# Tencent/PocketFlow

Hardware: AMD Instinct MI355X
Metric: images/sec ResNet-50 INT8 quant-aware fine-tune (whole job; per GPU = value / n_gpus) (higher is better)
Workload: dtype bf16

## Files before the change

### include/pocketflow_hip.h

```cpp
#ifndef POCKETFLOW_HIP_H_
#define POCKETFLOW_HIP_H_

#include <stdint.h>

#ifdef __cplusplus
extern "C" {
#endif

enum { PF_F32 = 0, PF_BF16 = 1 };
enum { PF_ACT_NONE = 0, PF_ACT_RELU = 1, PF_ACT_RELU6 = 2 };
enum { PF_BUCKET_TENSOR = 0, PF_BUCKET_CHANNEL = 1, PF_BUCKET_SPLIT = 2 };

typedef struct PfSeg {
  int64_t offset;
  int64_t len;
  int32_t RS;
  int32_t layout;
  int32_t I, O;
  int32_t mode;
  int32_t bits;
  int32_t bucket_size;
  int32_t n_bucket;
  int64_t slot_offset;
  int64_t cb_offset;
// ... 17 lines not shown
                void* stream);

int pf_seg_minmax(const float* w_flat, const PfSeg* segs, const PfBlock* blocks, int n_blocks,
                  uint32_t* slots, void* stream);
int pf_seg_uq_apply(const float* w_flat, void* qw_flat, int out_dtype, const PfSeg* segs,
                    const PfBlock* blocks, int n_blocks, const uint32_t* slots, void* stream);

int pf_seg_nuq_apply(const float* w_flat, void* qw_flat, int out_dtype, uint8_t* idx_flat,
                     const float* codebooks, const PfSeg* segs, const PfBlock* blocks,
                     int n_blocks, const uint32_t* slots, void* stream);
int pf_seg_nuq_codebook_grad(const void* g_flat, int g_dtype, const uint8_t* idx_flat,
                             float* dcodebooks, int64_t* acc_ws, int64_t n_codebook, const PfSeg* segs,
                             const PfBlock* blocks, int n_blocks, const uint32_t* slots, void* stream);
int pf_seg_normalize(const float* w_flat, float* xn_out, const PfSeg* segs, int seg_index,
                     const uint32_t* slots, void* stream);

int pf_ws_bkup_merge_abs(const float* var, float* bkup, const float* mask, float* abs_out,
                         int64_t n, void* stream);
int pf_kth_largest_nonneg(const float* a, int64_t n, int64_t k_desc_index, float* out,
                          uint32_t* workspace, void* stream);
int pf_ws_mask_apply(float* var, const float* bkup, float* mask, const float* thr, int64_t n,
                     void* stream);
int pf_count_nonzero(const float* x, int64_t n, unsigned long long* out, void* stream);

int pf_cp_build_mask(float* mask, const uint8_t* keep_in, const uint8_t* keep_out, int O, int RS,
                     int I, void* stream);
int pf_cp_mask_grad(float* g, const uint8_t* keep_in, const uint8_t* keep_out, int O, int RS,
                    int I, void* stream);

int pf_adam_flat(float* p, const void* g, int g_dtype, float* m, float* v, const float* mask,
                 int64_t n, int64_t n_decay, float wd, float g_scale, float lr, float beta1,
                 float beta2, float eps, float beta1_power, float beta2_power, void* stream);
int pf_momentum_flat(float* p, const void* g, int g_dtype, float* acc, const float* mask,
                     int64_t n, int64_t n_decay, float wd, float g_scale, float lr, float momentum,
                     void* stream);
int pf_adam_flat_dev(float* p, const void* g, int g_dtype, float* m, float* v, const float* mask,
                     int64_t n, int64_t n_decay, float wd, float g_scale, const float* hp, float beta1,
                     float beta2, float eps, void* stream);
int pf_momentum_flat_dev(float* p, const void* g, int g_dtype, float* acc, const float* mask,
                         int64_t n, int64_t n_decay, float wd, float g_scale, const float* hp,
                         float momentum, void* stream);
int pf_set_floats(float* dst, float a, float b, float c, float d, void* stream);

int pf_ce_distill_fwd_bwd(const void* z_s, int zs_dtype, const float* labels, const void* z_t,
                          int zt_dtype, int B, int C, float tempr, float loss_w, float* losses,
                          void* dz_s, int dz_dtype, float* row_ws, void* stream);

int pf_bn_stats(const void* x, int dtype, int64_t rows, int C, float* partial ,
                int n_blocks, void* stream);
int pf_bn_finalize(const float* partial, int n_blocks, int64_t rows, int C, const void* x_row0,
                   int dtype, const float* gamma, const float* beta, float* moving_mean,
                   float* moving_var, float momentum, float eps, int training ,
                   int act, float* scale_shift , float* mean_invstd ,
                   uint32_t* slot , void* stream);
int pf_bn_act_quant_apply(const void* x, void* q, int dtype, int64_t rows, int C,
                          const float* scale_shift, int act, const uint32_t* slot, int bits,
                          int quantize, void* stream);
int pf_bn_bwd_stats(const void* dq, const void* x, int dtype, int64_t rows, int C,
                    const float* scale_shift, const float* mean_invstd, int act,
                    float* partial , int n_blocks, void* stream);
int pf_bn_bwd_finalize(const float* partial, int n_blocks, int C, float* dgamma, float* dbeta,
                       void* stream);
int pf_bn_bwd_apply(const void* dq, const void* x, void* dx, int dtype, int64_t rows, int C,
                    const float* scale_shift, const float* mean_invstd,
                    const float* dgamma, const float* dbeta, int act, void* stream);
int pf_bn_bwd_apply_add(const void* dq, const void* x, const void* addend, void* dx, int dtype,
                        int64_t rows, int C, const float* scale_shift, const float* mean_invstd,
                        const float* dgamma, const float* dbeta, int act, void* stream);
int pf_bn_eval_scale_shift(const float* gamma, const float* beta, const float* moving_mean,
                           const float* moving_var, float eps, int C, float* scale_shift,
                           void* stream);

int pf_conv1x1_stats_groups(int M, int N);
int pf_conv1x1_stats_groups_k(int M, int N, int K, int prologue);
int pf_conv1x1_fwd(const void* X, const void* W, void* Y, const void* R, const float* scale_shift,
                   int act, const uint32_t* slot, int bits, float* partial, int M, int N, int K,
                   int Ho, int Wo, int H, int Wd, int stride, int ymap, void* stream);
int pf_conv1x1_fwd_affine(const void* X, const void* W, void* Y, const float* scale_shift, int act,
                          const float* out_scale_shift, int out_act, int M, int N, int K, int Ho, int Wo, int H, int Wd,
                          int stride, void* stream);
int pf_conv1x1_bwd_data_bnstats(const void* dY, const void* Wt, void* dQ, const void* bn_x,
                                const float* bn_scale_shift, const float* bn_mean_invstd, int bn_act,
                                float* partial, int M, int N, int K, void* stream);
int pf_conv1x1_wrw_splits(int M, int N, int K);
int pf_conv1x1_wrw(const void* dY, const void* X, void* dW, int dw_dtype, float* workspace,
                   const float* scale_shift, int act, const uint32_t* slot, int bits, int M, int N,
                   int K, int Ho, int Wo, int H, int Wd, int stride, void* stream);

int pf_conv2d_stats_groups(int M, int N);
int pf_conv2d_stats_groups_geom(int imgs, int H, int Wd, int C, int N, int th, int tw, int stride, int pad_h, int pad_w,
                                int Ho, int Wo);
int pf_conv2d_fwd(const void* X, const void* W, void* Y, const void* zero, const void* R, float* partial,
                  const void* bn_x, const float* bn_scale_shift, const float* bn_mean_invstd, int bn_act,
                  int imgs, int H, int Wd, int C, int N, int th, int tw, int stride, int pad_h, int pad_w,
                  int Ho, int Wo, void* stream);
int pf_conv2d_fwd_affine(const void* X, const void* W, void* Y, const void* zero, const float* out_scale_shift, int out_act,
                         int imgs, int H, int Wd, int C, int N, int th, int tw, int stride, int pad_h, int pad_w, int Ho, int Wo,
                         void* stream);

int pf_conv2d_wrw_splits(int M, int N, int C, int taps);
int pf_conv2d_wrw(const void* dY, const void* X, void* dW, int dw_dtype, float* workspace, int imgs, int H, int Wd, int C,
                  int N, int th, int tw, int stride, int pad_h, int pad_w, int Ho, int Wo, void* stream);

typedef struct PfTransposeTile {
  int64_t src_off, dst_off;
  int32_t O, I, src_ld, dst_ld;
  int32_t o0, i0;
  int32_t reserved0, reserved1;
} PfTransposeTile;
int pf_seg_transpose(const void* src_flat, void* dst_flat, int dtype, const void* tiles, int n_tiles, void* stream);

int pf_maxpool_fwd(const void* x, void* y, void* idx, int dtype, int B, int H, int W, int C, int k, int stride,
                   int pad_h, int pad_w, int Ho, int Wo, void* stream);
int pf_maxpool_bwd(const void* dy, const void* idx, void* dx, int dtype, int B, int H, int W, int C, int k, int stride,
                   int pad_h, int pad_w, int Ho, int Wo, void* stream);

int pf_conv_stem_supported(int H, int Wd, int C, int N, int k, int stride, int pad);
int pf_conv_stem_fwd(const void* X, const void* W, void* Y, int imgs, int H, int Wd, void* stream);
int pf_conv_stem_wrw_slabs(int imgs, int H, int Wd);
int pf_conv_stem_wrw(const void* dY, const void* X, void* dW, int dw_dtype, float* workspace, int imgs, int H, int Wd,
                     void* stream);

int pf_conv_stem3_supported(int H, int Wd, int C, int N, int k, int stride, int pad_h, int pad_w, int Ho, int Wo);
int pf_conv_stem3_fwd(const void* X, const void* W, void* Y, int imgs, int H, int Wd, int N, int pad_h, int pad_w, int Ho, int Wo,
                      void* stream);
int pf_conv_stem3_wrw_slabs(int imgs, int H, int Wd, int N, int pad_h, int pad_w, int Ho, int Wo);
int pf_conv_stem3_wrw(const void* dY, const void* X, void* dW, int dw_dtype, float* workspace, int imgs, int H, int Wd, int N,
                      int pad_h, int pad_w, int Ho, int Wo, void* stream);

int pf_depthwise_supported(int C, int k, int stride);
int pf_depthwise_groups(int B, int Ho, int Wo, int C);
int pf_depthwise_fwd(const void* X, const void* W, void* Y, int dtype, float* partial, int B, int H, int Wd, int C, int k,
                     int stride, int pad_h, int pad_w, int Ho, int Wo, void* stream);
int pf_depthwise_bwd_data(const void* dY, const void* W, void* dX, int dtype, int B, int H, int Wd, int C, int k,
                          int stride, int pad_h, int pad_w, int Ho, int Wo, void* stream);
int pf_depthwise_wrw(const void* dY, const void* X, void* dW, int dtype, int dw_dtype, float* slabs, int B, int H, int Wd,
                     int C, int k, int stride, int pad_h, int pad_w, int Ho, int Wo, void* stream);

typedef struct PfImageDesc {
  int64_t offset;
  int32_t h, w;
  float scale_y, scale_x;
  int32_t off_y, off_x;
  int32_t flip;
  int32_t reserved;
} PfImageDesc;
int pf_image_resize_bilinear(const void* src, const PfImageDesc* desc, void* out, int out_dtype, int B, int OH,
                             int OW, float mean_r, float mean_g, float mean_b, void* stream);

int pf_conv2d_bwd_data_strided(const void* dY, const void* Wt, void* dX, const void* zero, int imgs, int H, int Wd, int C, int N,
                               int R, int S, int stride, int pad_h, int pad_w, int Ho, int Wo, void* stream);
int pf_conv2d_bwd_data_strided_stats_groups(int imgs, int H, int Wd, int C, int stride);
int pf_conv2d_bwd_data_strided_bnstats(const void* dY, const void* Wt, void* dX, const void* zero, const void* bn_x,
                                       const float* bn_scale_shift, const float* bn_mean_invstd, int bn_act, float* partial,
                                       int imgs, int H, int Wd, int C, int N, int R, int S, int stride, int pad_h, int pad_w,
                                       int Ho, int Wo, void* stream);

int pf_convg_small_splits(int M, int Nc, int K);
int pf_convg_fwd(const void* x, const void* w, const float* bias, void* y, int dtype, int imgs, int H, int W, int C, int N, int R,
                 int S, int stride, int pad_h, int pad_w, int Ho, int Wo, float* slab, int64_t slab_elems, void* stream);
int pf_convg_bwd_data(const void* dy, const void* w, void* dx, int dtype, int imgs, int H, int W, int C, int N, int R, int S,
                      int stride, int pad_h, int pad_w, int Ho, int Wo, float* slab, int64_t slab_elems, void* stream);
int pf_convg_wrw_splits(int imgs, int C, int N, int R, int S, int Ho, int Wo);
int pf_convg_wrw(const void* dy, const void* x, void* dw, int dtype, int dw_dtype, float* slab, int imgs, int H, int W, int C, int N,
                 int R, int S, int stride, int pad_h, int pad_w, int Ho, int Wo, void* stream);

// ... 32 lines not shown
```

### pocketflow_amd/csrc/pf_conv.hip

```cpp
#include "pf_conv_common.h"

template <int BN_T, bool PRO, bool BWD, bool MAP>
__global__ __launch_bounds__(PF_THREADS, 2) void k_conv1x1_fwd(const ConvArgs a) {
  constexpr int WM = (BN_T == 128) ? 64 : 32;
  constexpr int JM = WM / 16;
  constexpr int CS_LD = BN_T + 8;
  constexpr int VPR = BN_T / 8;
  constexpr int RPP = PF_THREADS / VPR;
  constexpr int NBV = BN_T * 8 / PF_THREADS;
  constexpr int A_EL = CV_BM * CV_LDK, B_EL = BN_T * CV_LDK;
  constexpr int C_EL = CV_BM * CS_LD;
  constexpr int RED_FL = 4 * RPP * BN_T;
  constexpr int SM_BYTES_AB = (A_EL + B_EL) * 2;
  constexpr int SM_BYTES = SM_BYTES_AB > RED_FL * 4 ? (SM_BYTES_AB > C_EL * 2 ? SM_BYTES_AB : C_EL * 2)
                                                    : RED_FL * 4;
  constexpr int SS_BYTES = PRO ? 2 * CV_MAXK * 4 : 0;
  __shared__ __attribute__((aligned(16))) unsigned char smem[SM_BYTES + SS_BYTES];
  float* ssl = reinterpret_cast<float*>(smem + SM_BYTES);
  __shared__ float bpl[BWD ? 4 * BN_T : 4];
  bf16_t* As = reinterpret_cast<bf16_t*>(smem);
  bf16_t* Bs = As + A_EL;
  bf16_t* Cs = reinterpret_cast<bf16_t*>(smem);
  float* red = reinterpret_cast<float*>(smem);

// ... 165 lines not shown
      const int rl = wrow + p * RPP;
      const int m = m0 + rl, n = n0 + wvec * 8;
      if (m < a.M && n < a.N) {
        uint4 c = *reinterpret_cast<const uint4*>(Cs + rl * CS_LD + wvec * 8);
        const int64_t orow = (MAP && a.ymap) ? map_row(a, m) : (int64_t)m;
        if (bwd_stats) {
          float f[8], xv[8];
          unpack8(c, f);
          unpack8(rres[p], xv);
          const float* bp = bpl + wvec * 8;
#pragma unroll
          for (int j = 0; j < 8; ++j) {
            const float u = fmaf(bp[j], xv[j], bp[BN_T + j]);
            const float dy = (u > a.b_lo && u < a.b_hi) ? f[j] : 0.f;
            st_s[j] += dy;
            st_q[j] = fmaf(dy, (xv[j] - bp[2 * BN_T + j]) * bp[3 * BN_T + j], st_q[j]);
          }
        } else if (a.R != nullptr || a.partial != nullptr) {
          float f[8];
          unpack8(c, f);
          if (a.partial != nullptr) {
#pragma unroll
            for (int j = 0; j < 8; ++j) {
              st_s[j] += f[j];
              st_q[j] = fmaf(f[j], f[j], st_q[j]);
              st_mn[j] = pf_acc_min(st_mn[j], f[j]);
              st_mx[j] = pf_acc_max(st_mx[j], f[j]);
            }
          }
        }
        *reinterpret_cast<uint4*>(a.Y + orow * a.N + n) = c;
      }
    }
    __syncthreads();
  };

  for (int it = 0; it < total; it += 2) {
    body(it, ra0, av0);
    if (it + 1 < total) body(it + 1, ra1, av1);
  }

  if (a.partial != nullptr) {
    __syncthreads();
#pragma unroll
    for (int j = 0; j < 8; ++j) {
      red[(0 * RPP + wrow) * BN_T + wvec * 8 + j] = st_s[j];
      red[(1 * RPP + wrow) * BN_T + wvec * 8 + j] = st_q[j];
      red[(2 * RPP + wrow) * BN_T + wvec * 8 + j] = st_mn[j];
      red[(3 * RPP + wrow) * BN_T + wvec * 8 + j] = st_mx[j];
    }
    __syncthreads();
    const int nstat = bwd_stats ? 2 : 4;
    for (int t = tid; t < nstat * BN_T; t += PF_THREADS) {
      const int stat = t / BN_T, c = t - stat * BN_T;
      float v = red[(stat * RPP) * BN_T + c];
      for (int r = 1; r < RPP; ++r) {
        const float w = red[(stat * RPP + r) * BN_T + c];
        v = (stat < 2) ? (v + w) : (stat == 2 ? fminf(v, w) : fmaxf(v, w));
      }
      if (n0 + c < a.N) a.partial[((int64_t)g * nstat + stat) * a.N + n0 + c] = v;
    }
  }
}

#include <stdlib.h>
static int conv_bn_of(int N) {
  if (pf_tuning().conv_bn == 64) return 64;
  return (N % 128 == 0) ? 128 : 64;
}

static int conv_fwd_grid(int tiles_m, int tiles_n, int* G_out) {
  int G = 512 / tiles_n;
  G = (G / 8) * 8;
  if (G < 8) G = 8;
  const int need = ((tiles_m + 7) / 8) * 8;
  if (G > need) G = need;
  *G_out = G;
  return G * tiles_n;
}

int pf_conv_stream_plan(int M, int N, int K, int* nw_out);
int pf_conv_stream_groups(int nsplit);
int pf_conv_stream_launch(const ConvArgs& a, bool pro, bool bwd, hipStream_t st);

extern "C" int pf_conv1x1_stats_groups(int M, int N) {
  const int bn = conv_bn_of(N);
  int G;
  conv_fwd_grid((M + CV_BM - 1) / CV_BM, (N + bn - 1) / bn, &G);
  return G;
}

extern "C" int pf_conv2d_stats_groups(int M, int N);
int pf_igemm_stats_groups(int M, int N, int pro);
int pf_igemm_conv1x1(const void* X, const void* W, void* Y, const void* R, float* partial, const void* bn_x,
                     const float* bss, const float* bmi, float b_lo, float b_hi, const float* scale_shift,
                     const uint32_t* slot, float kq, float act_lo, float act_hi, int M, int N, int K, int Ho, int Wo,
                     int H, int Wd, int stride, const float* oss, int oact, hipStream_t st, int ymap = 0);
#ifndef PF_CONV_IGEMM_PLAIN_MINK
#define PF_CONV_IGEMM_PLAIN_MINK 256
#endif
static bool conv_use_igemm(bool pro, int K) {
  if ((pro ? pf_tuning().conv_igemm_pro : pf_tuning().conv_igemm) == 0) return false;
  return (K % 64) == 0 && (pro || K >= PF_CONV_IGEMM_PLAIN_MINK);
}

extern "C" int pf_conv1x1_stats_groups_k(int M, int N, int K, int prologue) {
  int nw = 0;
  const int nsplit = pf_conv_stream_plan(M, N, K, &nw);
  if (nsplit > 0) return pf_conv_stream_groups(nsplit);
  if (conv_use_igemm(prologue != 0, K)) return pf_igemm_stats_groups(M, N, prologue != 0);
  return pf_conv1x1_stats_groups(M, N);
}

static int conv_fwd_launch(const void* X, const void* W, void* Y, const void* R, const float* scale_shift,
                           int act, const uint32_t* slot, int bits, float* partial, int M, int N, int K,
                           int Ho, int Wo, int H, int Wd, int stride, int ymap, const void* bx,
                           const float* bss, const float* bmi, int bact, void* stream, const float* oss = nullptr,
                           int oact = PF_ACT_NONE) {
  if (oss != nullptr && (R != nullptr || partial != nullptr || bx != nullptr || ymap)) return (int)hipErrorInvalidValue;
  if (M <= 0 || N <= 0 || K <= 0 || (K % 8) || (N % 8)) return (int)hipErrorInvalidValue;
  if (!pf_aligned16(X) || !pf_aligned16(W) || !pf_aligned16(Y) || (R && !pf_aligned16(R)))
    return (int)hipErrorInvalidValue;
  if (slot != nullptr && (bits < 1 || bits > 32 || scale_shift == nullptr)) return (int)hipErrorInvalidValue;
  if (scale_shift != nullptr && K > CV_MAXK) return (int)hipErrorInvalidValue;
  if (stride < 1 || (stride > 1 && (Ho <= 0 || Wo <= 0 || H <= 0 || Wd <= 0))) return (int)hipErrorInvalidValue;
  ConvArgs a;
  a.X = (const bf16_t*)X; a.W = (const bf16_t*)W; a.Y = (bf16_t*)Y; a.R = (const bf16_t*)R;
  a.ss = scale_shift; a.slot = slot; a.partial = partial;
  a.kq = uq_k_of_bits(slot ? bits : 8);
  a.act_lo = (act == PF_ACT_NONE) ? -INFINITY : 0.0f;
  a.act_hi = (act == PF_ACT_RELU6) ? 6.0f : INFINITY;
  a.M = M; a.N = N; a.K = K;
  a.Ho = Ho; a.Wo = Wo; a.H = H; a.Wd = Wd; a.stride = stride; a.ymap = ymap; a.rows_per_split = 0;
  a.bx = (const bf16_t*)bx; a.bss = bss; a.bmi = bmi;
  a.b_lo = (bact == PF_ACT_NONE) ? -INFINITY : 0.0f;
  a.b_hi = (bact == PF_ACT_RELU6) ? 6.0f : INFINITY;
  a.oss = oss; a.oact = oact;
  if (bx != nullptr && (R != nullptr || partial == nullptr || bss == nullptr || bmi == nullptr || stride != 1 ||
                        !pf_aligned16(bx)))
    return (int)hipErrorInvalidValue;
  const int bn = conv_bn_of(N);
  a.tiles_m = (M + CV_BM - 1) / CV_BM;
  a.tiles_n = (N + bn - 1) / bn;
  const int grid = conv_fwd_grid(a.tiles_m, a.tiles_n, &a.G);
  hipStream_t st = (hipStream_t)stream;
  const bool pro = scale_shift != nullptr;
  if (bx != nullptr && pro) return (int)hipErrorInvalidValue;
  {
    const int r = pf_conv_stream_launch(a, pro, bx != nullptr, st);
    if (r >= 0) return r;
  }
  if (!ymap && conv_use_igemm(pro, K)) {
    const int r = pf_igemm_conv1x1(X, W, Y, R, partial, bx, bss, bmi, a.b_lo, a.b_hi, scale_shift, slot, a.kq, a.act_lo,
                                   a.act_hi, M, N, K, Ho, Wo, H, Wd, stride, oss, oact, st);
    if (r >= 0) return r;
  }
  if (ymap && stride > 1 && !pro && bx == nullptr && R == nullptr && partial == nullptr && oss == nullptr && conv_use_igemm(false, K) &&
      (N % 64) == 0) {
    const int r = pf_igemm_conv1x1(X, W, Y, nullptr, nullptr, nullptr, nullptr, nullptr, a.b_lo, a.b_hi, nullptr, nullptr, a.kq, a.act_lo,
                                   a.act_hi, M, N, K, Ho, Wo, H, Wd, stride, nullptr, PF_ACT_NONE, st, 1);
    if (r >= 0) return r;
  }
  if (oss != nullptr) {
    const int r = conv_fwd_launch(X, W, Y, R, scale_shift, act, slot, bits, partial, M, N, K, Ho, Wo, H, Wd, stride, ymap, bx, bss,
                                  bmi, bact, stream);
    if (r != 0) return r;
    return pf_bn_act_quant_apply(Y, Y, PF_BF16, M, N, oss, oact, nullptr, 8, 0, stream);
  }
  const bool map = stride != 1;
#define PF_CV(BNV)                                                                             \
  do {                                                                                         \
    if (pro) { if (map) k_conv1x1_fwd<BNV, true, false, true><<<grid, PF_THREADS, 0, st>>>(a);  \
               else k_conv1x1_fwd<BNV, true, false, false><<<grid, PF_THREADS, 0, st>>>(a); }   \
    else if (bx != nullptr) k_conv1x1_fwd<BNV, false, true, false><<<grid, PF_THREADS, 0, st>>>(a); \
    else { if (map) k_conv1x1_fwd<BNV, false, false, true><<<grid, PF_THREADS, 0, st>>>(a);     \
           else k_conv1x1_fwd<BNV, false, false, false><<<grid, PF_THREADS, 0, st>>>(a); }      \
  } while (0)
  if (bn == 128) PF_CV(128); else PF_CV(64);
#undef PF_CV
  PF_LAUNCH_CHECK();
  return 0;
}

extern "C" int pf_conv1x1_fwd(const void* X, const void* W, void* Y, const void* R, const float* scale_shift,
                              int act, const uint32_t* slot, int bits, float* partial, int M, int N, int K,
                              int Ho, int Wo, int H, int Wd, int stride, int ymap, void* stream) {
  return conv_fwd_launch(X, W, Y, R, scale_shift, act, slot, bits, partial, M, N, K, Ho, Wo, H, Wd, stride, ymap,
                         nullptr, nullptr, nullptr, PF_ACT_NONE, stream);
}

extern "C" int pf_conv1x1_fwd_affine(const void* X, const void* W, void* Y, const float* scale_shift, int act,
                                     const float* out_scale_shift, int out_act, int M, int N, int K, int Ho, int Wo, int H,
                                     int Wd, int stride, void* stream) {
  if (out_scale_shift == nullptr) return (int)hipErrorInvalidValue;
  return conv_fwd_launch(X, W, Y, nullptr, scale_shift, act, nullptr, 8, nullptr, M, N, K, Ho, Wo, H, Wd, stride, 0,
                         nullptr, nullptr, nullptr, PF_ACT_NONE, stream, out_scale_shift, out_act);
}

extern "C" int pf_conv1x1_bwd_data_bnstats(const void* dY, const void* Wt, void* dQ, const void* bn_x,
                                           const float* bn_scale_shift, const float* bn_mean_invstd, int bn_act,
                                           float* partial, int M, int N, int K, void* stream) {
  return conv_fwd_launch(dY, Wt, dQ, nullptr, nullptr, PF_ACT_NONE, nullptr, 8, partial, M, K, N, 0, 0, 0, 0, 1, 0,
                         bn_x, bn_scale_shift, bn_mean_invstd, bn_act, stream);
}

#define WR_TN 128
#define WR_TK 64
#define WR_BM 64
#define WR_LDM (WR_BM + 8)

__device__ __forceinline__ void st_transposed(bf16_t* S, int c0, int m, const uint4& v) {
  const uint32_t w[4] = {v.x, v.y, v.z, v.w};
  const int mg = m >> 3, ml = m & 7;
#pragma unroll
  for (int j = 0; j < 8; ++j) {
    const int c = c0 + j;
    S[c * WR_LDM + (((mg ^ ((c >> 3) & 7)) << 3) | ml)] = (bf16_t)((w[j >> 1] >> ((j & 1) * 16)) & 0xFFFFu);
  }
}

template <bool PRO>
__global__ __launch_bounds__(PF_THREADS, 2) void k_conv1x1_wrw(const ConvArgs a) {
  __shared__ __attribute__((aligned(16))) bf16_t Ds[WR_TN * WR_LDM];
  __shared__ __attribute__((aligned(16))) bf16_t Qs[WR_TK * WR_LDM];
  const int ntile = gridDim.x, nwg = gridDim.x * gridDim.y;
  int wg = blockIdx.y * gridDim.x + blockIdx.x;
  {
    const int xcd = wg & 7, idx = wg >> 3;
    const int q = nwg >> 3, r = nwg & 7;
    wg = (xcd < r ? xcd * (q + 1) : r * (q + 1) + (xcd - r) * q) + idx;
  }
  const int tile = wg % ntile, split = wg / ntile;
  const int tn = tile % a.tiles_n, tk = tile / a.tiles_n;
  const int n0 = tn * WR_TN, k0 = tk * WR_TK;
  const int mbeg = split * a.rows_per_split;
  const int mend = (mbeg + a.rows_per_split < a.M) ? (mbeg + a.rows_per_split) : a.M;
  const int tid = threadIdx.x, wave = tid >> 6, lane = tid & 63;
  const int frow = lane & 15, fm = lane >> 4;

  Pro pro;
  pro_init(pro, a.act_lo, a.act_hi, a.kq, PRO ? a.slot : nullptr);
  const int qkp = tid & 7;
  if (PRO) {
    const int k = k0 + qkp * 8;
    if (k < a.K) {
#pragma unroll
      for (int j = 0; j < 8; ++j) { pro.sc[j] = pro_fold_scale(pro, a.ss[k + j]); pro.sh[j] = pro_fold_shift(pro, a.ss[a.K + k + j]); }
    }
  }
  f32x4 acc[2][4];
#pragma unroll
  for (int i = 0; i < 2; ++i)
#pragma unroll
    for (int j = 0; j < 4; ++j) acc[i][j] = (f32x4){0.f, 0.f, 0.f, 0.f};

  uint4 rd[4], rq[2];
  bool vq[2];
  auto gload = [&](int mb) {
#pragma unroll
    for (int i = 0; i < 4; ++i) {
      const int p = tid + i * PF_THREADS;
      const int m = mb + (p >> 4), n = n0 + (p & 15) * 8;
      uint4 v = make_uint4(0, 0, 0, 0);
      if (m < mend && n < a.N) v = *reinterpret_cast<const uint4*>(a.W + (int64_t)m * a.N + n);
      rd[i] = v;
    }
#pragma unroll
    for (int i = 0; i < 2; ++i) {
      const int p = tid + i * PF_THREADS;
      const int m = mb + (p >> 3), k = k0 + (p & 7) * 8;
      uint4 v = make_uint4(0, 0, 0, 0);
      vq[i] = (m < mend && k < a.K);
      if (vq[i]) v = *reinterpret_cast<const uint4*>(a.X + map_row(a, m) * a.K + k);
      rq[i] = v;
    }
  };
  auto sstore = [&]() {
#pragma unroll
    for (int i = 0; i < 4; ++i) {
      const int p = tid + i * PF_THREADS;
      st_transposed(Ds, (p & 15) * 8, p >> 4, rd[i]);
    }
#pragma unroll
    for (int i = 0; i < 2; ++i) {
      const int p = tid + i * PF_THREADS;
      uint4 v = rq[i];
// ... 151 lines not shown
```

### pocketflow_amd/csrc/pf_conv_common.h

```cpp
#pragma once
#include "pf_common.h"

typedef __attribute__((ext_vector_type(8))) __bf16 bf16x8;
typedef __attribute__((ext_vector_type(4))) float f32x4;

#define CV_BM 128
#define CV_BK 64
#define CV_LDK (CV_BK + 8)
#define CV_MAXK 2048

typedef __attribute__((ext_vector_type(2))) __bf16 bf16x2_t;
typedef __attribute__((ext_vector_type(2))) float f32x2_t;
__device__ __forceinline__ uint32_t pack_bf16x2(float a, float b) {
  const f32x2_t v = {a, b};
  const bf16x2_t r = __builtin_convertvector(v, bf16x2_t);
  return *reinterpret_cast<const uint32_t*>(&r);
}
__device__ __forceinline__ void unpack8(const uint4& v, float* o) {
  o[0] = __uint_as_float(v.x << 16); o[1] = __uint_as_float(v.x & 0xFFFF0000u);
  o[2] = __uint_as_float(v.y << 16); o[3] = __uint_as_float(v.y & 0xFFFF0000u);
  o[4] = __uint_as_float(v.z << 16); o[5] = __uint_as_float(v.z & 0xFFFF0000u);
  o[6] = __uint_as_float(v.w << 16); o[7] = __uint_as_float(v.w & 0xFFFF0000u);
}
__device__ __forceinline__ uint4 pack8(const float* o) {
  return make_uint4(pack_bf16x2(o[0], o[1]), pack_bf16x2(o[2], o[3]), pack_bf16x2(o[4], o[5]),
                    pack_bf16x2(o[6], o[7]));
}

struct ConvArgs {
  const bf16_t* X;
  const bf16_t* W;
  bf16_t* Y;
  const bf16_t* R;
  const float* ss;
  const uint32_t* slot;
  float* partial;
  float kq, act_lo, act_hi;
  int M, N, K;
  int tiles_m, tiles_n, G;
  int Ho, Wo, H, Wd, stride;
  int ymap;
  int rows_per_split;
  const bf16_t* bx;
  const float* bss;
  const float* bmi;
  float b_lo, b_hi;
  const float* oss;
  int oact;
};

__device__ __forceinline__ uint4 out_affine8(const uint4& c, const float* __restrict__ oss, int N, int n, int act) {
  float f[8];
  unpack8(c, f);
  const float4 s0 = *reinterpret_cast<const float4*>(oss + n), s1 = *reinterpret_cast<const float4*>(oss + n + 4);
  const float4 h0 = *reinterpret_cast<const float4*>(oss + N + n), h1 = *reinterpret_cast<const float4*>(oss + N + n + 4);
  const float sc[8] = {s0.x, s0.y, s0.z, s0.w, s1.x, s1.y, s1.z, s1.w};
  const float sh[8] = {h0.x, h0.y, h0.z, h0.w, h1.x, h1.y, h1.z, h1.w};
#pragma unroll
  for (int j = 0; j < 8; ++j) {
    float y = fmaf(sc[j], f[j], sh[j]);
    if (act != PF_ACT_NONE) y = fmaxf(y, 0.f);
    if (act == PF_ACT_RELU6) y = fminf(y, 6.f);
    f[j] = y;
  }
  return pack8(f);
}

__device__ __forceinline__ int64_t map_row(const ConvArgs& a, int m) {
  if (a.stride == 1) return m;
  const int hw = a.Ho * a.Wo;
  const int n = m / hw, rem = m - n * hw;
  const int ho = rem / a.Wo, wo = rem - ho * a.Wo;
  return ((int64_t)n * a.H + (int64_t)ho * a.stride) * a.Wd + (int64_t)wo * a.stride;
}

struct Pro {
  float sc[8], sh[8];
  float lo, hi;
  float beta, c1, c2;
  int quant;
};
__device__ __forceinline__ void pro_init(Pro& p, float act_lo, float act_hi, float kq, const uint32_t* slot) {
  p.quant = 0; p.beta = 0.f; p.c1 = 1.f; p.c2 = 1.f;
  if (slot != nullptr) {
    float alpha, beta;
    slot_alpha_beta(slot, alpha, beta);
    p.quant = 1; p.beta = beta; p.c1 = kq / alpha; p.c2 = alpha / kq;
  }
  p.lo = (act_lo - p.beta) * p.c1;
  p.hi = (act_hi - p.beta) * p.c1;
}
__device__ __forceinline__ float pro_fold_scale(const Pro& p, float scale) { return scale * p.c1; }
__device__ __forceinline__ float pro_fold_shift(const Pro& p, float shift) { return (shift - p.beta) * p.c1; }
__device__ __forceinline__ float pro_point(const Pro& p, float sc, float sh, float x) {
  const float t = __builtin_amdgcn_fmed3f(fmaf(sc, x, sh), p.lo, p.hi);
  return p.quant ? fmaf(rintf(t), p.c2, p.beta) : t;
}
__device__ __forceinline__ uint4 pro_apply_scalar(const Pro& p, const uint4& v) {
  float f[8];
  unpack8(v, f);
#pragma unroll
  for (int j = 0; j < 8; ++j) f[j] = pro_point(p, p.sc[j], p.sh[j], f[j]);
  return pack8(f);
}
typedef float f32x2p_t __attribute__((ext_vector_type(2)));
__device__ __forceinline__ uint4 pro_apply(const Pro& p, const uint4& v) {
  const uint32_t w[4] = {v.x, v.y, v.z, v.w};
  uint32_t o[4];
  if (p.quant) {
    const f32x2p_t c2 = {p.c2, p.c2}, be = {p.beta, p.beta};
#pragma unroll
    for (int i = 0; i < 4; ++i) {
      const f32x2p_t x = {__uint_as_float(w[i] << 16), __uint_as_float(w[i] & 0xFFFF0000u)};
      const f32x2p_t sc = {p.sc[2 * i], p.sc[2 * i + 1]}, sh = {p.sh[2 * i], p.sh[2 * i + 1]};
      const f32x2p_t t = __builtin_elementwise_fma(sc, x, sh);
      const f32x2p_t r = {rintf(__builtin_amdgcn_fmed3f(t[0], p.lo, p.hi)), rintf(__builtin_amdgcn_fmed3f(t[1], p.lo, p.hi))};
      const f32x2p_t q = __builtin_elementwise_fma(r, c2, be);
      o[i] = pack_bf16x2(q[0], q[1]);
    }
  } else {
#pragma unroll
    for (int i = 0; i < 4; ++i) {
      const f32x2p_t x = {__uint_as_float(w[i] << 16), __uint_as_float(w[i] & 0xFFFF0000u)};
      const f32x2p_t sc = {p.sc[2 * i], p.sc[2 * i + 1]}, sh = {p.sh[2 * i], p.sh[2 * i + 1]};
      const f32x2p_t t = __builtin_elementwise_fma(sc, x, sh);
      o[i] = pack_bf16x2(__builtin_amdgcn_fmed3f(t[0], p.lo, p.hi), __builtin_amdgcn_fmed3f(t[1], p.lo, p.hi));
    }
  }
  return make_uint4(o[0], o[1], o[2], o[3]);
}

__device__ __forceinline__ uint32_t lds_addr(const void* p) { return (uint32_t)(uintptr_t)p; }
// ... 57 lines not shown
```

### pocketflow_amd/csrc/pf_conv_stream.hip

```cpp
#include "pf_conv_common.h"
#include <stdlib.h>

#define ST_THREADS 512
#define ST_WAVES 8
#define ST_GRID 256

template <int NW, bool PRO, bool BWD, bool MAP, bool AFF = false>
__global__ __launch_bounds__(ST_THREADS) void k_conv1x1_stream(const ConvArgs a, const int nsplit) {
  constexpr int JM = (NW == 256) ? 1 : 2;
  constexpr int RS = 16 * JM;
  constexpr int NI = NW / 16;
  constexpr int D = (NW == 128) ? 2 : 4;
  constexpr int CS_LD = NW + 8;
  constexpr int VPR = NW / 8;
  constexpr int RPP = 64 / VPR;
  constexpr int NP = RS / RPP;
  constexpr int NR = 2 * JM;

  extern __shared__ __attribute__((aligned(16))) unsigned char smem[];
  const int K = a.K, KC = K >> 6, KV = K >> 3;
  bf16_t* Wl = reinterpret_cast<bf16_t*>(smem);
  float* aux = reinterpret_cast<float*>(smem + (size_t)NW * K * 2);
  const int aux_fl = PRO ? 2 * K : (BWD ? 4 * NW : 0);
  bf16_t* Cs_all = reinterpret_cast<bf16_t*>(smem + (size_t)NW * K * 2 + (size_t)aux_fl * 4);
  float* red = reinterpret_cast<float*>(Cs_all);

  const int tid = threadIdx.x, wave = tid >> 6, lane = tid & 63;
  const int l15 = lane & 15, q = lane >> 4;
  bf16_t* Cs = Cs_all + wave * (RS * CS_LD);

  const int xcd = blockIdx.x & 7, idx = blockIdx.x >> 3;
  const int slice = idx % nsplit, g = (idx / nsplit) * 8 + xcd;
  const int nsets = gridDim.x / nsplit;
  const int n0 = slice * NW;
  const int sstep = nsets * ST_WAVES;
  const int NS = (a.M + RS - 1) / RS;
  const int s_first = g * ST_WAVES + wave;
  const int cnt = (s_first < NS) ? (NS - s_first + sstep - 1) / sstep : 0;
  const int T = cnt * KC;

  Pro pro;
  pro_init(pro, a.act_lo, a.act_hi, a.kq, PRO ? a.slot : nullptr);
  {
    const int swz_mask = (KV >= 16) ? 15 : 7;
    for (int v = tid; v < NW * KV; v += ST_THREADS) {
      const int n = v / KV, c = v - n * KV;
      uint4 w = make_uint4(0, 0, 0, 0);
      if (n0 + n < a.N) w = *reinterpret_cast<const uint4*>(a.W + (int64_t)(n0 + n) * K + c * 8);
      *reinterpret_cast<uint4*>(Wl + ((int64_t)n * KV + (c ^ (n & swz_mask))) * 8) = w;
    }
    if (PRO) for (int i = tid; i < 2 * K; i += ST_THREADS)
      aux[i] = (i < K) ? pro_fold_scale(pro, a.ss[i]) : pro_fold_shift(pro, a.ss[i]);
    if (BWD) for (int i = tid; i < 4 * NW; i += ST_THREADS) {
      const int qq = i / NW, c = n0 + (i - qq * NW);
      float v = 0.f;
      if (c < a.N) v = (qq < 2) ? a.bss[qq * a.N + c] : a.bmi[(qq - 2) * a.N + c];
      aux[i] = v;
    }
  }
  __syncthreads();

  const int wswz = (KV >= 16) ? l15 : (l15 & 7);
  const bf16_t* __restrict__ side = BWD ? a.bx : nullptr;
  const bool has_r = !BWD && a.R != nullptr;
  const int wvec = lane % VPR, wrow = lane / VPR;

  f32x4 acc[NI][JM];
  uint4 ring[D][NR];
  uint4 rres[NP];
  uint2 rr[NI][JM];
  float st_s[8], st_q[8], st_mn[8], st_mx[8];
#pragma unroll
  for (int j = 0; j < 8; ++j) { st_s[j] = 0.f; st_q[j] = 0.f; st_mn[j] = INFINITY; st_mx[j] = -INFINITY; }

  int ld_s = s_first, ld_kc = 0;
  auto issue = [&](uint4 (&r)[NR]) {
#pragma unroll
    for (int j = 0; j < JM; ++j) {
      int m = ld_s * RS + j * 16 + l15;
      m = (m < a.M) ? m : (a.M - 1);
      const int64_t row = (!MAP || a.ymap) ? (int64_t)m : map_row(a, m);
      const bf16_t* p = a.X + row * K + ld_kc * 64 + q * 8;
      r[j * 2 + 0] = *reinterpret_cast<const uint4*>(p);
      r[j * 2 + 1] = *reinterpret_cast<const uint4*>(p + 32);
    }
    if (++ld_kc == KC) { ld_kc = 0; ld_s += sstep; }
  };
  auto issue_side = [&](int s, int p) {
    const int m = s * RS + p * RPP + wrow, n = n0 + wvec * 8;
    uint4 v = make_uint4(0, 0, 0, 0);
    if (m < a.M && n < a.N) {
      const int64_t orow = (MAP && a.ymap) ? map_row(a, m) : (int64_t)m;
      v = *reinterpret_cast<const uint4*>(side + orow * a.N + n);
    }
    rres[p] = v;
  };

  auto issue_res = [&](int s) {
#pragma unroll
    for (int j = 0; j < JM; ++j) {
      const int m = s * RS + j * 16 + l15;
      const int64_t orow = (m < a.M) ? ((MAP && a.ymap) ? map_row(a, m) : (int64_t)m) : 0;
#pragma unroll
      for (int i = 0; i < NI; ++i) {
        const int n = n0 + i * 16 + q * 4;
        uint2 v = make_uint2(0, 0);
        if (m < a.M && n < a.N) v = *reinterpret_cast<const uint2*>(a.R + orow * a.N + n);
        rr[i][j] = v;
      }
    }
  };
#pragma clang loop unroll(full)
  for (int d = 0; d < D; ++d)
    if (d < T) issue(ring[d]);
  if (has_r && cnt > 0) issue_res(s_first);
  if (side != nullptr && cnt > 0) {
#pragma unroll
    for (int p = 0; p < NP; ++p) issue_side(s_first, p);
  }

  int cs = s_first, ckc = 0;
  int slot = 0;
  for (int t = 0; t < T; ++t) {
    uint4 v[NR];
    const bool refill = t + D < T;
#pragma clang loop unroll(full)
    for (int d = 0; d < D; ++d) {
      if (slot == d) {
#pragma unroll
        for (int i = 0; i < NR; ++i) v[i] = ring[d][i];
        if (refill) issue(ring[d]);
      }
    }
    slot = (slot + 1 == D) ? 0 : slot + 1;
    if (ckc == 0) {
#pragma unroll
      for (int i = 0; i < NI; ++i)
#pragma unroll
        for (int j = 0; j < JM; ++j) acc[i][j] = (f32x4){0.f, 0.f, 0.f, 0.f};
    }
#pragma unroll
    for (int kk = 0; kk < 2; ++kk) {
      if (PRO) {
        const int k = ckc * 64 + kk * 32 + q * 8;
        const float4 s0 = *reinterpret_cast<const float4*>(aux + k), s1 = *reinterpret_cast<const float4*>(aux + k + 4);
        const float4 h0 = *reinterpret_cast<const float4*>(aux + K + k), h1 = *reinterpret_cast<const float4*>(aux + K + k + 4);
        pro.sc[0] = s0.x; pro.sc[1] = s0.y; pro.sc[2] = s0.z; pro.sc[3] = s0.w;
        pro.sc[4] = s1.x; pro.sc[5] = s1.y; pro.sc[6] = s1.z; pro.sc[7] = s1.w;
        pro.sh[0] = h0.x; pro.sh[1] = h0.y; pro.sh[2] = h0.z; pro.sh[3] = h0.w;
        pro.sh[4] = h1.x; pro.sh[5] = h1.y; pro.sh[6] = h1.z; pro.sh[7] = h1.w;
      }
      bf16x8 xf[JM];
#pragma unroll
      for (int j = 0; j < JM; ++j) {
        uint4 u = v[j * 2 + kk];
        if (PRO) u = (NW == 128) ? pro_apply_scalar(pro, u) : pro_apply(pro, u);
        xf[j] = *reinterpret_cast<const bf16x8*>(&u);
      }
      const int c = (ckc * 8 + kk * 4 + q) ^ wswz;
      constexpr int WB = 4;
#pragma unroll
      for (int ib = 0; ib < NI; ib += WB) {
        bf16x8 wf[WB];
#pragma unroll
        for (int i = 0; i < WB; ++i)
          wf[i] = *reinterpret_cast<const bf16x8*>(Wl + ((int64_t)((ib + i) * 16 + l15) * KV + c) * 8);
#pragma unroll
        for (int i = 0; i < WB; ++i)
#pragma unroll
          for (int j = 0; j < JM; ++j)
            acc[ib + i][j] = __builtin_amdgcn_mfma_f32_16x16x32_bf16(wf[i], xf[j], acc[ib + i][j], 0, 0, 0);
      }
      if (PRO) __builtin_amdgcn_sched_group_barrier(0x100, 4, 0);
      constexpr int DEPTH = (NW == 128) ? 2 : 4;
      __builtin_amdgcn_sched_group_barrier(0x100, DEPTH, 0);
#pragma unroll
      for (int i = 0; i < NI - DEPTH; ++i) {
        __builtin_amdgcn_sched_group_barrier(0x008, JM, 0);
        __builtin_amdgcn_sched_group_barrier(0x100, 1, 0);
      }
      __builtin_amdgcn_sched_group_barrier(0x008, DEPTH * JM, 0);
    }
    const bool last = (ckc == KC - 1);
    const int s = cs;
    if (++ckc == KC) { ckc = 0; cs += sstep; }
    if (!last) continue;

    if (has_r) {
#pragma unroll
      for (int i = 0; i < NI; ++i)
#pragma unroll
        for (int j = 0; j < JM; ++j) {
          acc[i][j][0] += __uint_as_float(rr[i][j].x << 16); acc[i][j][1] += __uint_as_float(rr[i][j].x & 0xFFFF0000u);
          acc[i][j][2] += __uint_as_float(rr[i][j].y << 16); acc[i][j][3] += __uint_as_float(rr[i][j].y & 0xFFFF0000u);
        }
    }
#pragma unroll
    for (int i = 0; i < NI; ++i)
#pragma unroll
      for (int j = 0; j < JM; ++j) {
        const uint2 w = make_uint2(pack_bf16x2(acc[i][j][0], acc[i][j][1]), pack_bf16x2(acc[i][j][2], acc[i][j][3]));
        *reinterpret_cast<uint2*>(Cs + (j * 16 + l15) * CS_LD + i * 16 + q * 4) = w;
      }
    const bool more = (cs < NS);
    if (has_r && more) issue_res(cs);
    float bpr[32];
    if (BWD && NW != 128) {
#pragma unroll
      for (int qq = 0; qq < 4; ++qq)
#pragma unroll
        for (int j = 0; j < 8; ++j) bpr[qq * 8 + j] = aux[qq * NW + wvec * 8 + j];
    } else if (BWD) {
#pragma unroll
      for (int i = 0; i < 32; ++i) bpr[i] = 0.f;
    }
    constexpr int CB = (NW == 128) ? 1 : 4;
    uint4 cv[CB];
#pragma unroll
    for (int p = 0; p < NP; ++p) {
      const int rl = p * RPP + wrow;
      const int m = s * RS + rl, n = n0 + wvec * 8;
      if (p % CB == 0) {
#pragma unroll
        for (int pb = 0; pb < CB; ++pb)
          if (p + pb < NP) cv[pb] = *reinterpret_cast<const uint4*>(Cs + ((p + pb) * RPP + wrow) * CS_LD + wvec * 8);
      }
      uint4 c = cv[p % CB];
      const uint4 sv = rres[p];
      if (side != nullptr && more) issue_side(cs, p);
      if (m < a.M && n < a.N) {
        const int64_t orow = (MAP && a.ymap) ? map_row(a, m) : (int64_t)m;
        if (BWD) {
          float f[8], xv[8];
          unpack8(c, f);
          unpack8(sv, xv);
          const float* bp = (NW == 128) ? (aux + wvec * 8) : bpr;
          constexpr int BPS = (NW == 128) ? NW : 8;
#pragma unroll
          for (int j = 0; j < 8; ++j) {
            const float u = fmaf(bp[j], xv[j], bp[BPS + j]);
            const float dy = (u > a.b_lo && u < a.b_hi) ? f[j] : 0.f;
            st_s[j] += dy;
            st_q[j] = fmaf(dy, (xv[j] - bp[2 * BPS + j]) * bp[3 * BPS + j], st_q[j]);
          }
        } else if (a.R != nullptr || a.partial != nullptr) {
          float f[8];
          unpack8(c, f);
          if (a.partial != nullptr) {
#pragma unroll
            for (int j = 0; j < 8; ++j) {
              st_s[j] += f[j];
              st_q[j] = fmaf(f[j], f[j], st_q[j]);
              st_mn[j] = pf_acc_min(st_mn[j], f[j]);
              st_mx[j] = pf_acc_max(st_mx[j], f[j]);
            }
          }
        }
        if constexpr (AFF) c = out_affine8(c, a.oss, a.N, n, a.oact);
        *reinterpret_cast<uint4*>(a.Y + orow * a.N + n) = c;
      }
    }
  }

  if (a.partial != nullptr) {
#pragma unroll
    for (int o = VPR; o < 64; o <<= 1) {
#pragma unroll
      for (int j = 0; j < 8; ++j) {
        st_s[j] += __shfl_xor(st_s[j], o, 64);
        st_q[j] += __shfl_xor(st_q[j], o, 64);
        st_mn[j] = fminf(st_mn[j], __shfl_xor(st_mn[j], o, 64));
        st_mx[j] = fmaxf(st_mx[j], __shfl_xor(st_mx[j], o, 64));
      }
    }
    __syncthreads();
    if (lane < VPR) {
#pragma unroll
      for (int j = 0; j < 8; ++j) {
        red[(0 * ST_WAVES + wave) * NW + lane * 8 + j] = st_s[j];
        red[(1 * ST_WAVES + wave) * NW + lane * 8 + j] = st_q[j];
        red[(2 * ST_WAVES + wave) * NW + lane * 8 + j] = st_mn[j];
        red[(3 * ST_WAVES + wave) * NW + lane * 8 + j] = st_mx[j];
      }
    }
    __syncthreads();
    const int nstat = BWD ? 2 : 4;
    for (int t = tid; t < nstat * NW; t += ST_THREADS) {
      const int stat = t / NW, c = t - stat * NW;
      float v = red[(stat * ST_WAVES) * NW + c];
      for (int w = 1; w < ST_WAVES; ++w) {
        const float x = red[(stat * ST_WAVES + w) * NW + c];
        v = (stat < 2) ? (v + x) : (stat == 2 ? fminf(v, x) : fmaxf(v, x));
      }
      if (n0 + c < a.N) a.partial[((int64_t)g * nstat + stat) * a.N + n0 + c] = v;
    }
  }
}

static int stream_enabled() {
  return pf_tuning().conv_stream;
}

static int stream_max_split() {
  return pf_tuning().conv_stream_maxsplit;
}

int pf_conv_stream_plan(int M, int N, int K, int* nw_out) {
  if (!stream_enabled()) return 0;
  if ((K % 64) || K > 512 || (N % 64) || N > 2048) return 0;
  if (M < 4096) return 0;
  int nsplit = 1;
  while ((int64_t)(N / nsplit) * K > 32768 || N / nsplit > 256) nsplit *= 2;
  const int nw = N / nsplit;
  if (nsplit > stream_max_split() || (ST_GRID % (8 * nsplit)) || (nw != 64 && nw != 128 && nw != 256)) return 0;
  if (nsplit >= 2 && N < 4 * K) return 0;
  *nw_out = nw;
  return nsplit;
}

int pf_conv_stream_groups(int nsplit) { return ST_GRID / nsplit; }

template <int NW, bool PRO, bool BWD, bool MAP, bool AFF = false>
static int stream_launch_t(const ConvArgs& a, int nsplit, hipStream_t st) {
  const int JM = (NW == 256) ? 1 : 2, RS = 16 * JM;
  const size_t aux_fl = PRO ? 2 * (size_t)a.K : (BWD ? 4 * (size_t)NW : 0);
  const size_t lds = (size_t)NW * a.K * 2 + aux_fl * 4 + (size_t)ST_WAVES * RS * (NW + 8) * 2;
  if (int e = pf_require_lds(reinterpret_cast<const void*>(&k_conv1x1_stream<NW, PRO, BWD, MAP, AFF>), lds)) return e;
  k_conv1x1_stream<NW, PRO, BWD, MAP, AFF><<<ST_GRID, ST_THREADS, lds, st>>>(a, nsplit);
  PF_LAUNCH_CHECK();
  return 0;
}

int pf_conv_stream_launch(const ConvArgs& a, bool pro, bool bwd, hipStream_t st) {
  int nw = 0;
  const int nsplit = pf_conv_stream_plan(a.M, a.N, a.K, &nw);
  if (nsplit == 0) return -1;
  const bool map = a.stride != 1;
  if (a.oss != nullptr) {
    if (map || bwd) return -1;
#define PF_STA(NWV) do { return pro ? stream_launch_t<NWV, true, false, false, true>(a, nsplit, st)     \
                                    : stream_launch_t<NWV, false, false, false, true>(a, nsplit, st); } while (0)
    if (nw == 64) PF_STA(64);
    if (nw == 128) PF_STA(128);
    PF_STA(256);
#undef PF_STA
  }
#define PF_ST(NWV)                                                                                  \
  do {                                                                                              \
    if (pro) return map ? stream_launch_t<NWV, true, false, true>(a, nsplit, st)                    \
                        : stream_launch_t<NWV, true, false, false>(a, nsplit, st);                  \
    if (bwd) return stream_launch_t<NWV, false, true, false>(a, nsplit, st);                        \
    return map ? stream_launch_t<NWV, false, false, true>(a, nsplit, st)                            \
               : stream_launch_t<NWV, false, false, false>(a, nsplit, st);                          \
  } while (0)
  if (nw == 64) PF_ST(64);
  if (nw == 128) PF_ST(128);
  PF_ST(256);
#undef PF_ST
}
```

### pocketflow_amd/csrc/pf_igemm.h

```cpp
#pragma once
#include "pf_conv_common.h"

#define LDS_PTR(p) ((__attribute__((address_space(3))) void*)(p))

#if defined(__HIP_DEVICE_COMPILE__)
typedef __amdgpu_buffer_rsrc_t pf_rsrc_t;
#define PF_MAKE_RSRC(p, bytes) __builtin_amdgcn_make_buffer_rsrc((void*)(p), (short)0, (int)(bytes), 0x00020000)
#define PF_BUFFER_LOAD_LDS16(rs, lds, voff, soff) __builtin_amdgcn_raw_ptr_buffer_load_lds(rs, LDS_PTR(lds), 16, voff, soff, 0, 0)
#else
typedef int pf_rsrc_t;
#define PF_MAKE_RSRC(p, bytes) 0
#define PF_BUFFER_LOAD_LDS16(rs, lds, voff, soff) ((void)(rs), (void)(lds), (void)(voff), (void)(soff))
#endif

struct IgArgs {
  const bf16_t* X;
  const bf16_t* W;
  bf16_t* Y;
  const bf16_t* zero;
  uint32_t x_bytes, w_bytes;
  const bf16_t* R;
  float* partial;
  const bf16_t* bx;
  const float* bss;
  const float* bmi;
  float b_lo, b_hi;
  const float* ss;
  const uint32_t* slot;
  float kq, act_lo, act_hi;
  int M, N, C;
  int th, tw;
  int H, Wd, Ho, Wo, stride, pad_h, pad_w;
  int tiles_m, tiles_n, G;
  int w_r0, w_rs, w_s0, w_ss, w_S, w_taps_full;
  int o_sub, o_y, o_x, o_H, o_W;
  const float* oss;
  int oact;
};

template <int N> __device__ __forceinline__ void wait_vm() { asm volatile("s_waitcnt vmcnt(%0)" ::"n"(N) : "memory"); }

#define IG_PLAIN 0
#define IG_BWD 1
#define IG_PRO 2
```

### pocketflow_amd/csrc/pf_igemm.hip

```cpp
#include "pf_conv_common.h"
#include <stdio.h>
#include <stdlib.h>

#include "pf_igemm.h"

#ifndef PF_IG_ABLATE
#define PF_IG_ABLATE 0
#endif
#define PF_IG_NO_DMA (PF_IG_ABLATE == 2 || PF_IG_ABLATE == 3 || PF_IG_ABLATE == 4)
#define PF_IG_FAKE_FRAGS (PF_IG_ABLATE == 3 || PF_IG_ABLATE == 4)

#ifdef PF_IG_TIMING
#define PF_IG_STAMP(k) do { if (tm_tile == 2) tmk[k] = (uint32_t)__builtin_readcyclecounter(); } while (0)
#else
#define PF_IG_STAMP(k) do { } while (0)
#endif

#ifdef PF_IG_CODES
#define PF_IG_XB 1
__device__ __forceinline__ bf16x8 ig_codes_to_bf16x8(uint2 c) {
  uint32_t r[4];
#pragma unroll
  for (int h = 0; h < 2; ++h) {
    const uint32_t w = h ? c.y : c.x;
    const float f0 = (float)(w & 0xffu), f1 = (float)((w >> 8) & 0xffu), f2 = (float)((w >> 16) & 0xffu), f3 = (float)(w >> 24);
    r[h * 2 + 0] = __builtin_amdgcn_perm(__float_as_uint(f1), __float_as_uint(f0), 0x07060302u);
    r[h * 2 + 1] = __builtin_amdgcn_perm(__float_as_uint(f3), __float_as_uint(f2), 0x07060302u);
  }
  const uint4 u = make_uint4(r[0], r[1], r[2], r[3]);
  return *reinterpret_cast<const bf16x8*>(&u);
}
#else
#define PF_IG_XB 2
#endif

template <int BM, int BN, int WM, int WN, int NS, int MODE, bool SUB = false, bool AFF = false>
__global__ __launch_bounds__(64 * WM * WN) void k_igemm(const IgArgs a) {
  constexpr bool BWD = (MODE == IG_BWD), PRO = (MODE == IG_PRO);
  static_assert(!PRO || NS == 2 || NS == 3, "the in-LDS prologue pass is written for the 2- and 3-stage rings");
  constexpr bool PRO3 = PRO && NS == 3;
  constexpr int NWC = WM * WN;
  constexpr int T = 64 * NWC;
  constexpr int TS = T;
  constexpr int TE = T;
  constexpr int WR = BM / WM, WC = BN / WN;
  constexpr int JM = WR / 16, NI = WC / 16;
  constexpr int XB = PF_IG_XB;
  constexpr int ACH = 4 * XB, AROW = 64 * XB;
  constexpr int AS = BM * ACH / TS, BS = BN * 8 / TS;
  constexpr int A_BYTES = BM * AROW, B_BYTES = BN * 128, STAGE = A_BYTES + B_BYTES;
  constexpr int CS_LD = BN + 8, CS_LD_B = BN + 8;
  constexpr int VPR = BN / 8, RPP = TE / VPR, NP = BM / RPP;
  static_assert(AS >= 1 && BS >= 1 && NP >= 1, "tile too small for the block");
  constexpr int LPS = AS + BS;
  extern __shared__ __attribute__((aligned(16))) unsigned char smem[];
  bf16_t* Cs = reinterpret_cast<bf16_t*>(smem);
  float* red = reinterpret_cast<float*>(smem);
  constexpr int RING_B = NS * STAGE, CT_B = BM * CS_LD_B * 2;
  float* bpl = reinterpret_cast<float*>(smem + (RING_B > CT_B ? RING_B : CT_B));
  float* ssl = bpl;

  const int tid = threadIdx.x, lane = tid & 63;
  const int wave = __builtin_amdgcn_readfirstlane(tid >> 6);
  const int swave = wave;
  const int cwave = wave % NWC;
  const int wm = cwave / WN, wn = cwave % WN;
  const int l15 = lane & 15, q = lane >> 4;
  const int srow = (swave * 64 + lane) >> 3;
  const int schunk = (lane & 7) ^ ((lane >> 3) & 7);
  const int srowA = (XB == 2) ? srow : ((swave * 64 + lane) >> 2);
  const int schunkA = (XB == 2) ? schunk : ((lane & 3) ^ ((lane >> 4) & 3));

  const int xcd = blockIdx.x & 7, L = blockIdx.x >> 3;
  const int g = xcd + 8 * (L / a.tiles_n), tn = L % a.tiles_n;
  const int n0 = tn * BN;
  const int cch = a.C >> 6;
  const int taps = a.th * a.tw;
  const int nk = taps * cch;
  const int64_t wrow = (int64_t)(SUB ? a.w_taps_full : taps) * a.C;
  const int hw_o = a.Ho * a.Wo;

  if (BWD) {
    for (int i = tid; i < 4 * BN; i += T) {
      const int qq = i / BN, c = n0 + (i - qq * BN);
      float v = 0.f;
      if (c < a.N) v = (qq < 2) ? a.bss[qq * a.N + c] : a.bmi[(qq - 2) * a.N + c];
      bpl[i] = v;
    }
  }

  float st_s[8], st_q[8], st_mn[8], st_mx[8];
#pragma unroll
  for (int j = 0; j < 8; ++j) { st_s[j] = 0.f; st_q[j] = 0.f; st_mn[j] = INFINITY; st_mx[j] = -INFINITY; }
  const int wvec = tid % VPR, wrw = tid / VPR;
  const bf16_t* __restrict__ side = BWD ? a.bx : nullptr;
  Pro pro;
  pro_init(pro, a.act_lo, a.act_hi, a.kq, PRO ? a.slot : nullptr);
  if (PRO3) {
    for (int i = tid; i < 2 * a.C; i += T) ssl[i] = (i < a.C) ? pro_fold_scale(pro, a.ss[i]) : pro_fold_shift(pro, a.ss[i]);
    __syncthreads();
  }

  const pf_rsrc_t rsX = PF_MAKE_RSRC(a.X, a.x_bytes);
  const pf_rsrc_t rsW = PF_MAKE_RSRC(a.W, a.w_bytes);
  constexpr uint32_t OOB = 0x80000000u;
  uint32_t boff[BS];
#pragma unroll
  for (int i = 0; i < BS; ++i) {
    const int n = n0 + i * (TS / 8) + srow;
    boff[i] = (n < a.N) ? (uint32_t)(((int64_t)n * wrow + schunk * 8) * 2) : OOB;
  }

  const bool pointwise = a.th == 1 && a.tw == 1 && a.stride == 1 && a.pad_h == 0 && a.pad_w == 0 && a.Ho == a.H && a.Wo == a.Wd;
  constexpr bool XPRE = !BWD && NS == 3 && 2 * STAGE >= BM * CS_LD_B * 2;
  constexpr int RB0 = XPRE ? 2 : 0;
  uint32_t pbase[AS], pmask[AS];
  int s_r = 0, s_s = 0, s_cc = 0, s_ks = 0, s_tap = 0;
  auto setup_tile = [&](int m0) {
#pragma unroll
    for (int i = 0; i < AS; ++i) {
      const int m = m0 + i * (TS / ACH) + srowA;
      pbase[i] = 0; pmask[i] = 0;
      if (pointwise) {
        if (m < a.M) { pbase[i] = (uint32_t)(m * a.C + schunkA * (16 / XB)) * (uint32_t)XB; pmask[i] = 1u; }
      } else if (m < a.M) {
        const int img = m / hw_o, rem = m - img * hw_o;
        const int ho = rem / a.Wo, wo = rem - ho * a.Wo;
        const int h0 = ho * a.stride - a.pad_h, w0 = wo * a.stride - a.pad_w;
        pbase[i] = (uint32_t)(((img * a.H + h0) * a.Wd + w0) * a.C + schunkA * (16 / XB)) * (uint32_t)XB;
        uint32_t mk = 0;
        for (int r = 0; r < a.th; ++r)
          for (int sx = 0; sx < a.tw; ++sx)
            if ((unsigned)(h0 + r) < (unsigned)a.H && (unsigned)(w0 + sx) < (unsigned)a.Wd) mk |= 1u << (r * a.tw + sx);
        pmask[i] = mk;
      }
    }
    s_r = 0; s_s = 0; s_cc = 0; s_ks = 0; s_tap = 0;
  };
  auto stage = [&](int buf) {
    unsigned char* As = smem + buf * STAGE;
    unsigned char* Bs = As + A_BYTES;
    const uint32_t tapoff = (uint32_t)(((s_r * a.Wd + s_s) * a.C + s_cc * 64) * XB);
#if !PF_IG_NO_DMA
#pragma unroll
    for (int i = 0; i < AS; ++i) {
      const uint32_t voff = ((pmask[i] >> s_tap) & 1u) ? (pbase[i] + tapoff) : OOB;
      PF_BUFFER_LOAD_LDS16(rsX, As + (i * (TS / ACH) + swave * (64 / ACH)) * AROW, voff, 0);
    }
    uint32_t woff = (uint32_t)(s_ks * 128);
    if constexpr (SUB) woff = (uint32_t)((((a.w_r0 + s_r * a.w_rs) * a.w_S + a.w_s0 + s_s * a.w_ss) * a.C + s_cc * 64) * 2);
#pragma unroll
    for (int i = 0; i < BS; ++i)
      PF_BUFFER_LOAD_LDS16(rsW, Bs + (i * (TS / 8) + swave * 8) * 128, boff[i], woff);
#else
    (void)As; (void)Bs; (void)tapoff;
#endif
    ++s_ks;
    if (++s_cc == cch) { s_cc = 0; ++s_tap; if (++s_s == a.tw) { s_s = 0; ++s_r; } }
  };
  bool pre = false;
#ifdef PF_IG_TIMING
  uint32_t tmk[16];
  int tm_tile = -1;
#pragma unroll
  for (int k = 0; k < 16; ++k) tmk[k] = 0;
#endif
  for (int tm = g; tm < a.tiles_m; tm += a.G) {
    const int m0 = tm * BM;
#ifdef PF_IG_TIMING
    ++tm_tile;
#endif
    PF_IG_STAMP(0);
    if (!pre) setup_tile(m0);

    f32x4 acc[NI][JM];
#pragma unroll
    for (int i = 0; i < NI; ++i)
#pragma unroll
      for (int j = 0; j < JM; ++j) acc[i][j] = (f32x4){0.f, 0.f, 0.f, 0.f};
    uint2 rr[NI][JM];
    const bool has_r = !BWD && a.R != nullptr;
    constexpr bool RPRE = BM * BN <= 128 * 256;
    auto load_residual = [&]() {
#pragma unroll
      for (int j = 0; j < JM; ++j) {
        const int m = m0 + wm * WR + j * 16 + l15;
#pragma unroll
        for (int i = 0; i < NI; ++i) {
          const int n = n0 + wn * WC + i * 16 + q * 4;
          rr[i][j] = make_uint2(0, 0);
          if (m < a.M && n < a.N) rr[i][j] = *reinterpret_cast<const uint2*>(a.R + (int64_t)m * a.N + n);
        }
      }
    };
    auto add_residual = [&](auto& c) {
#pragma unroll
      for (int j = 0; j < JM; ++j)
#pragma unroll
        for (int i = 0; i < NI; ++i) {
          c[i][j][0] += __uint_as_float(rr[i][j].x << 16); c[i][j][1] += __uint_as_float(rr[i][j].x & 0xFFFF0000u);
          c[i][j][2] += __uint_as_float(rr[i][j].y << 16); c[i][j][3] += __uint_as_float(rr[i][j].y & 0xFFFF0000u);
        }
    };

    int ibuf = RB0;
    float4 ps0 = make_float4(0, 0, 0, 0), ps1 = ps0, ph0 = ps0, ph1 = ps0;
    auto fetch_ss = [&](int cc) {
      const float* p = a.ss + cc * 64 + schunk * 8;
      ps0 = *reinterpret_cast<const float4*>(p); ps1 = *reinterpret_cast<const float4*>(p + 4);
      ph0 = *reinterpret_cast<const float4*>(p + a.C); ph1 = *reinterpret_cast<const float4*>(p + a.C + 4);
    };
    auto transform3 = [&](int buf, int cc, int i0, int i1) {
      const uint32_t pss = lds_addr(ssl + cc * 64 + schunk * 8);
      float4 s0, s1, h0, h1;
      if (i1 - i0 == 1 || i1 - i0 == 2) {
        const uint32_t pd = lds_addr(smem + buf * STAGE + srow * 128 + (lane & 7) * 16) + (uint32_t)(i0 * (TS / 8) * 128);
        uint4 v0, v1 = make_uint4(0, 0, 0, 0);
        if (i1 - i0 == 1) lds_read_b128x4_1(pss, pss + (uint32_t)a.C * 4u, pd, s0, s1, h0, h1, v0);
        else lds_read_b128x4_2(pss, pss + (uint32_t)a.C * 4u, pd, pd + (TS / 8) * 128, s0, s1, h0, h1, v0, v1);
        pro.sc[0] = s0.x; pro.sc[1] = s0.y; pro.sc[2] = s0.z; pro.sc[3] = s0.w;
        pro.sc[4] = s1.x; pro.sc[5] = s1.y; pro.sc[6] = s1.z; pro.sc[7] = s1.w;
        pro.sh[0] = h0.x; pro.sh[1] = h0.y; pro.sh[2] = h0.z; pro.sh[3] = h0.w;
        pro.sh[4] = h1.x; pro.sh[5] = h1.y; pro.sh[6] = h1.z; pro.sh[7] = h1.w;
        lds_write_b128(pd, pro_apply(pro, v0));
        if (i1 - i0 == 2) lds_write_b128(pd + (TS / 8) * 128, pro_apply(pro, v1));
        return;
      }
      lds_read_b128x4(pss, pss + (uint32_t)a.C * 4u, s0, s1, h0, h1);
      pro.sc[0] = s0.x; pro.sc[1] = s0.y; pro.sc[2] = s0.z; pro.sc[3] = s0.w;
      pro.sc[4] = s1.x; pro.sc[5] = s1.y; pro.sc[6] = s1.z; pro.sc[7] = s1.w;
      pro.sh[0] = h0.x; pro.sh[1] = h0.y; pro.sh[2] = h0.z; pro.sh[3] = h0.w;
      pro.sh[4] = h1.x; pro.sh[5] = h1.y; pro.sh[6] = h1.z; pro.sh[7] = h1.w;
      const uint32_t pv = lds_addr(smem + buf * STAGE + srow * 128 + (lane & 7) * 16);
      static_assert(!PRO3 || AS == 1 || AS == 2 || AS == 4 || AS == 8, "vector count per lane");
#pragma unroll
      for (int i = 0; i < AS; i += 2) {
        if (i >= i0 && i < i1) {
          if (i + 1 < i1) {
            uint4 v0, v1;
            lds_read_b128x2(pv + i * (TS / 8) * 128, pv + (i + 1) * (TS / 8) * 128, v0, v1);
            lds_write_b128(pv + i * (TS / 8) * 128, pro_apply(pro, v0));
            lds_write_b128(pv + (i + 1) * (TS / 8) * 128, pro_apply(pro, v1));
          } else {
            lds_write_b128(pv + i * (TS / 8) * 128, pro_apply(pro, lds_read_b128(pv + i * (TS / 8) * 128)));
          }
        } else if (i + 1 >= i0 && i + 1 < i1) {
          lds_write_b128(pv + (i + 1) * (TS / 8) * 128, pro_apply(pro, lds_read_b128(pv + (i + 1) * (TS / 8) * 128)));
        }
      }
    };
    auto transform = [&](int buf) {
      const float rs[8] = {ps0.x, ps0.y, ps0.z, ps0.w, ps1.x, ps1.y, ps1.z, ps1.w};
      const float rh[8] = {ph0.x, ph0.y, ph0.z, ph0.w, ph1.x, ph1.y, ph1.z, ph1.w};
#pragma unroll
      for (int j = 0; j < 8; ++j) { pro.sc[j] = pro_fold_scale(pro, rs[j]); pro.sh[j] = pro_fold_shift(pro, rh[j]); }
      unsigned char* As = smem + buf * STAGE;
#pragma unroll
      for (int i = 0; i < AS; ++i) {
        uint4* p = reinterpret_cast<uint4*>(As + (i * (TS / 8) + srow) * 128 + (lane & 7) * 16);
        *p = pro_apply(pro, *p);
      }
    };
    {
#pragma unroll
    for (int d = 0; d < NS - 1; ++d)
      if (d < nk) {
        if (d > 0 || !pre) {
          if (PRO && !PRO3) fetch_ss(s_cc);
          stage(ibuf);
        }
        ibuf = (ibuf + 1 == NS) ? 0 : ibuf + 1;
      }
    PF_IG_STAMP(1);
    if (nk >= NS - 1) wait_vm<(NS - 2) * LPS>(); else wait_vm<0>();
// ... 22 lines not shown
#pragma unroll
      for (int kk = 0; kk < 2; ++kk) {
        const int coff = (((kk * 4 + q) ^ (l15 & 7)) << 4);
        bf16x8 wf[NI], xf[JM];
#if PF_IG_ABLATE != 1
#if PF_IG_FAKE_FRAGS
#pragma unroll
        for (int i = 0; i < NI; ++i) { uint4 u = make_uint4(lane, i, kk, 0x3f803f80u); asm volatile("" : "+v"(u.x)); wf[i] = *reinterpret_cast<const bf16x8*>(&u); }
#pragma unroll
        for (int j = 0; j < JM; ++j) { uint4 u = make_uint4(lane, j, kk, 0x3f803f80u); asm volatile("" : "+v"(u.x)); xf[j] = *reinterpret_cast<const bf16x8*>(&u); }
        (void)coff;
#else
#pragma unroll
        for (int i = 0; i < NI; ++i)
          wf[i] = *reinterpret_cast<const bf16x8*>(Bs + (wn * WC + i * 16 + l15) * 128 + coff);
#ifdef PF_IG_CODES
        const int coffA = ((((kk * 2 + (q >> 1)) ^ ((l15 >> 2) & 3)) << 4) + (q & 1) * 8);
#pragma unroll
        for (int j = 0; j < JM; ++j)
          xf[j] = ig_codes_to_bf16x8(*reinterpret_cast<const uint2*>(As + (wm * WR + j * 16 + l15) * AROW + coffA));
#else
#pragma unroll
        for (int j = 0; j < JM; ++j)
          xf[j] = *reinterpret_cast<const bf16x8*>(As + (wm * WR + j * 16 + l15) * 128 + coff);
#endif
#endif
#pragma unroll
        for (int i = 0; i < NI; ++i)
#pragma unroll
          for (int j = 0; j < JM; ++j)
            acc[i][j] = __builtin_amdgcn_mfma_f32_16x16x32_bf16(wf[i], xf[j], acc[i][j], 0, 0, 0);
        if constexpr (NI == 4 && JM == 4 && PRO3) {
          __builtin_amdgcn_sched_group_barrier(0x100, NI + JM, 0);
          __builtin_amdgcn_sched_group_barrier(0x008, NI * JM, 0);
        }
        if constexpr ((NI == 4 || NI == 2) && JM == 4 && !PRO3) {
          if (kk == 1) {
            __builtin_amdgcn_sched_group_barrier(0x100, NI + JM, 0);
#pragma unroll
            for (int i = 0; i < NI + JM; ++i) {
              __builtin_amdgcn_sched_group_barrier(0x008, (NI * JM) / (NI + JM), 0);
              __builtin_amdgcn_sched_group_barrier(0x100, 1, 0);
            }
            __builtin_amdgcn_sched_group_barrier(0x008, NI * JM - (NI + JM) * ((NI * JM) / (NI + JM)) + NI * JM, 0);
          }
        }
#else
        (void)coff; (void)wf; (void)xf;
#endif
        if (tnext) transform3(cbuf, ks + 1, kk * (AS / 2), (kk == 1) ? AS : (AS / 2));
      }
      if (!PRO3) {
        if (more) wait_vm<(NS - 2) * LPS>(); else wait_vm<0>();
      }
      if (PRO && !PRO3 && more) transform(tbuf);
      asm volatile("s_waitcnt lgkmcnt(0)" ::: "memory");
      __builtin_amdgcn_s_barrier();
      __builtin_amdgcn_sched_barrier(0);
#ifdef PF_IG_TIMING
      if (ks < 4) PF_IG_STAMP(4 + ks);
      if (ks == nk - 1) PF_IG_STAMP(8);
#endif
    }
    }

#if PF_IG_ABLATE >= 4
    {
      if (a.M < 0) {
#pragma unroll
        for (int i = 0; i < NI; ++i)
#pragma unroll
          for (int j = 0; j < JM; ++j) reinterpret_cast<uint32_t*>(a.Y)[(i * JM + j) * 64 + lane] = pack_bf16x2(acc[i][j][0] + acc[i][j][1], acc[i][j][2] + acc[i][j][3]);
      }
      continue;
    }
#endif
    {
    if (has_r) {
      if constexpr (RPRE) add_residual(acc);
      else {
#pragma unroll
        for (int j = 0; j < JM; ++j) {
          const int m = m0 + wm * WR + j * 16 + l15;
#pragma unroll
          for (int i = 0; i < NI; ++i) {
            const int n = n0 + wn * WC + i * 16 + q * 4;
            if (m < a.M && n < a.N) {
              const uint2 r = *reinterpret_cast<const uint2*>(a.R + (int64_t)m * a.N + n);
              acc[i][j][0] += __uint_as_float(r.x << 16); acc[i][j][1] += __uint_as_float(r.x & 0xFFFF0000u);
              acc[i][j][2] += __uint_as_float(r.y << 16); acc[i][j][3] += __uint_as_float(r.y & 0xFFFF0000u);
            }
          }
          __builtin_amdgcn_sched_barrier(0);
        }
      }
    }
    PF_IG_STAMP(9);
    pre = false;
    if constexpr (XPRE) {
      __builtin_amdgcn_sched_barrier(0);
      if (tm + a.G < a.tiles_m) {
        setup_tile((tm + a.G) * BM);
        stage(RB0);
        pre = true;
      }
      __builtin_amdgcn_sched_barrier(0);
    }
#ifdef PF_IG_CODES
#pragma unroll
    for (int i = 0; i < NI; ++i)
#pragma unroll
      for (int j = 0; j < JM; ++j)
#pragma unroll
        for (int e = 0; e < 4; ++e) acc[i][j][e] *= a.kq;
#endif
#pragma unroll
    for (int i = 0; i < NI; ++i)
#pragma unroll
      for (int j = 0; j < JM; ++j) {
        const uint2 v = make_uint2(pack_bf16x2(acc[i][j][0], acc[i][j][1]), pack_bf16x2(acc[i][j][2], acc[i][j][3]));
        if constexpr (XPRE) lds_write_b64(lds_addr(Cs + (wm * WR + j * 16 + l15) * CS_LD + wn * WC + i * 16 + q * 4), v);
        else *reinterpret_cast<uint2*>(Cs + (wm * WR + j * 16 + l15) * CS_LD + wn * WC + i * 16 + q * 4) = v;
      }
    }
    constexpr int PG = (NP > 8) ? 8 : NP;
    uint4 rres[PG];
    auto load_side = [&](int p0) {
#pragma unroll
      for (int p = 0; p < PG; ++p) {
        const int m = m0 + wrw + (p0 + p) * RPP, n = n0 + wvec * 8;
        rres[p] = make_uint4(0, 0, 0, 0);
        if (m < a.M && n < a.N) {
          int64_t srow = m;
          if constexpr (SUB) {
            const int oimg = m / hw_o, orem = m - oimg * hw_o;
            const int oi = orem / a.Wo, oj = orem - oi * a.Wo;
            srow = ((int64_t)oimg * a.o_H + oi * a.o_sub + a.o_y) * a.o_W + oj * a.o_sub + a.o_x;
          }
          rres[p] = *reinterpret_cast<const uint4*>(side + srow * a.N + n);
        }
      }
    };
    constexpr bool etid = true;
    float bpr[32];
    if (BWD) {
#pragma unroll
      for (int qq = 0; qq < 4; ++qq)
#pragma unroll
        for (int j = 0; j < 8; ++j) bpr[qq * 8 + j] = bpl[qq * BN + wvec * 8 + j];
    }
    if (side != nullptr && etid) load_side(0);
    PF_IG_STAMP(10);
    if constexpr (XPRE) { asm volatile("s_waitcnt lgkmcnt(0)" ::: "memory"); __builtin_amdgcn_s_barrier(); __builtin_amdgcn_sched_barrier(0); }
    else __syncthreads();
    PF_IG_STAMP(11);
#pragma unroll
    for (int p0 = 0; p0 < NP; p0 += PG) {
      u32x4_t cv[8];
      if constexpr (XPRE && PG == 8) {
#pragma unroll
        for (int pp = 0; pp < PG; ++pp) lds_read_b128_nowait(lds_addr(Cs + (wrw + (p0 + pp) * RPP) * CS_LD + wvec * 8), cv[pp]);
        lds_wait_batch8(cv);
      } else {
#pragma unroll
        for (int pp = 0; pp < PG; ++pp) cv[pp] = *reinterpret_cast<const u32x4_t*>(Cs + (wrw + (p0 + pp) * RPP) * CS_LD + wvec * 8);
      }
#pragma unroll
      for (int pp = 0; pp < PG; ++pp) {
        const int p = p0 + pp;
        const int rl = wrw + p * RPP;
        const int m = m0 + rl, n = n0 + wvec * 8;
        if (m < a.M && n < a.N && etid) {
          uint4 c;
          c = make_uint4(cv[pp][0], cv[pp][1], cv[pp][2], cv[pp][3]);
          if (BWD) {
            float f[8], xv[8];
            unpack8(c, f);
            unpack8(rres[pp], xv);
            const float* bp = bpr;
            constexpr int BPS = 8;
#pragma unroll
            for (int j = 0; j < 8; ++j) {
              const float u = fmaf(bp[j], xv[j], bp[BPS + j]);
              const float dy = (u > a.b_lo && u < a.b_hi) ? f[j] : 0.f;
              st_s[j] += dy;
              st_q[j] = fmaf(dy, (xv[j] - bp[2 * BPS + j]) * bp[3 * BPS + j], st_q[j]);
            }
          } else if (a.R != nullptr || a.partial != nullptr) {
            float f[8];
            unpack8(c, f);
            if (a.partial != nullptr) {
#pragma unroll
              for (int j = 0; j < 8; ++j) {
                st_s[j] += f[j];
                st_q[j] = fmaf(f[j], f[j], st_q[j]);
                st_mn[j] = pf_acc_min(st_mn[j], f[j]);
                st_mx[j] = pf_acc_max(st_mx[j], f[j]);
              }
            }
          }
          if constexpr (AFF) c = out_affine8(c, a.oss, a.N, n, a.oact);
          int64_t orow = m;
          if constexpr (SUB) {
            const int oimg = m / hw_o, orem = m - oimg * hw_o;
            const int oi = orem / a.Wo, oj = orem - oi * a.Wo;
            orow = ((int64_t)oimg * a.o_H + oi * a.o_sub + a.o_y) * a.o_W + oj * a.o_sub + a.o_x;
          }
          *reinterpret_cast<uint4*>(a.Y + orow * a.N + n) = c;
        }
      }
      if (side != nullptr && p0 + PG < NP && etid) load_side(p0 + PG);
    }
    PF_IG_STAMP(12);
    if constexpr (XPRE) { asm volatile("s_waitcnt lgkmcnt(0)" ::: "memory"); __builtin_amdgcn_s_barrier(); __builtin_amdgcn_sched_barrier(0); }
    else __syncthreads();
    PF_IG_STAMP(13);
#ifdef PF_IG_TIMING
    if (tm_tile == 2 && blockIdx.x == gridDim.x / 2 && tid == 0) {
      uint32_t* out = reinterpret_cast<uint32_t*>(const_cast<bf16_t*>(a.zero));
#pragma unroll
      for (int k = 0; k < 14; ++k) out[k] = tmk[k];
      out[14] = (uint32_t)__builtin_readcyclecounter();
    }
#endif
  }

  if (a.partial != nullptr) {
    constexpr int nstat_max = 4;
    const int nstat = BWD ? 2 : 4;
    __syncthreads();
    for (int stat = 0; stat < nstat; ++stat) {
      const float* v = (stat == 0) ? st_s : (stat == 1 ? st_q : (stat == 2 ? st_mn : st_mx));
#pragma unroll
      for (int j = 0; j < 8; ++j) red[wrw * BN + wvec * 8 + j] = v[j];
      __syncthreads();
      for (int c = tid; c < BN; c += T) {
        float r = red[c];
        for (int rr = 1; rr < RPP; ++rr) {
          const float w = red[rr * BN + c];
          r = (stat < 2) ? (r + w) : (stat == 2 ? fminf(r, w) : fmaxf(r, w));
        }
        if (n0 + c < a.N) a.partial[((int64_t)g * nstat + stat) * a.N + n0 + c] = r;
      }
      __syncthreads();
    }
    (void)nstat_max;
  }
}

struct IgCfg { int bm, bn, slots; bool pro3; };

static bool ig_pro3_enabled() {
  return pf_tuning().igemm_pro3 != 0;
}

static IgCfg ig_pick(int M, int N, bool pro) {
  if (pro) {
    if (ig_pro3_enabled()) {
      if (N % 256 == 0) return IgCfg{128, 256, 256, true};
      if (N % 128 == 0) return IgCfg{256, 128, 256, true};
    }
    return IgCfg{128, (N % 128 == 0) ? 128 : 64, 512, false};
  }
  {
    const int bm = pf_tuning().igemm_tile_bm, bn = pf_tuning().igemm_tile_bn;
    if ((bm == 128 || bm == 256) && (bn == 64 || bn == 128) && (N % bn == 0 || bn == 64))
      return IgCfg{bm, bn, (bm == 256) ? 256 : 512, false};
  }
  const int bn = (N % 128 == 0) ? 128 : 64;
  return IgCfg{128, bn, 512, false};
}

static int ig_grid(int slots, int tiles_m, int tiles_n, int* G_out) {
  int G = slots / tiles_n;
  G = (G / 8) * 8;
  if (G < 8) G = 8;
  const int need = ((tiles_m + 7) / 8) * 8;
  if (G > need) G = need;
  *G_out = G;
  return G * tiles_n;
}

int pf_igemm_stats_groups_geom(int M, int N, int pro, int taps, int C) {
  (void)taps; (void)C;
  const IgCfg c = ig_pick(M, N, pro != 0);
  int G;
  ig_grid(c.slots, (M + c.bm - 1) / c.bm, (N + c.bn - 1) / c.bn, &G);
  return G;
}

int pf_igemm_stats_groups(int M, int N, int pro) { return pf_igemm_stats_groups_geom(M, N, pro, 1, 64); }

extern "C" int pf_conv2d_stats_groups(int M, int N) { return pf_igemm_stats_groups(M, N, 0); }

template <int BM, int BN, int WM, int WN, int NS, int MODE, bool SUB = false, bool AFF = false>
static int ig_launch_t(IgArgs& a, int slots, hipStream_t st) {
  constexpr bool BWD = (MODE == IG_BWD), PRO3 = (MODE == IG_PRO && NS == 3);
  constexpr int THREADS = 64 * WM * WN;
  a.tiles_m = (a.M + BM - 1) / BM;
  a.tiles_n = (a.N + BN - 1) / BN;
  const int grid = ig_grid(slots, a.tiles_m, a.tiles_n, &a.G);
  constexpr size_t ring = NS * (size_t)(BM + BN) * 128, ctile = (size_t)BM * (BN + 8) * 2;
  constexpr size_t base = (ring > ctile ? ring : ctile);
  const size_t lds = base + (BWD ? 4 * BN * 4 : 0) + (PRO3 ? 2 * (size_t)a.C * 4 : 0);
  if (PRO3 && a.C > CV_MAXK) return (int)hipErrorInvalidValue;
  const size_t lds_max = base + (BWD ? 4 * BN * 4 : 0) + (PRO3 ? 2 * (size_t)CV_MAXK * 4 : 0);
  if (int e = pf_require_lds(reinterpret_cast<const void*>(&k_igemm<BM, BN, WM, WN, NS, MODE, SUB, AFF>), lds_max)) return e;
  k_igemm<BM, BN, WM, WN, NS, MODE, SUB, AFF><<<grid, THREADS, lds, st>>>(a);
  PF_LAUNCH_CHECK();
  return 0;
}

bool pf_conv3x3_c64_geom(int H, int Wd, int C, int N, int th, int tw, int stride, int pad_h, int pad_w, int Ho, int Wo);
bool pf_conv3x3_c64_takes(const IgArgs& a);
int pf_conv3x3_c64_stats_groups(int M);
int pf_conv3x3_c64_launch(const IgArgs& a, hipStream_t st);

static int ig_launch(IgArgs& a, hipStream_t st) {
  const bool bwd = a.bx != nullptr, pro = a.ss != nullptr;
  if (pf_conv3x3_c64_takes(a)) return pf_conv3x3_c64_launch(a, st);
  const IgCfg c = ig_pick(a.M, a.N, pro);
  if (a.oss != nullptr) {
    if (bwd) return (int)hipErrorInvalidValue;
    if (pro && c.pro3 && a.th * a.tw == 1)
      return (c.bn == 256) ? ig_launch_t<128, 256, 2, 4, 3, IG_PRO, false, true>(a, c.slots, st)
                           : ig_launch_t<256, 128, 4, 2, 3, IG_PRO, false, true>(a, c.slots, st);
    if (!pro && c.bm == 128 && c.bn == 128) return ig_launch_t<128, 128, 2, 2, 2, IG_PLAIN, false, true>(a, c.slots, st);
    if (!pro && c.bm == 128 && c.bn == 64) return ig_launch_t<128, 64, 2, 2, 2, IG_PLAIN, false, true>(a, c.slots, st);
    const float* oss = a.oss;
    a.oss = nullptr;
    const int r = ig_launch(a, st);
    if (r != 0) return r;
    return pf_bn_act_quant_apply(a.Y, a.Y, PF_BF16, a.M, a.N, oss, a.oact, nullptr, 8, 0, st);
  }
  if (pro) {
    if (a.th * a.tw != 1 || bwd) return (int)hipErrorInvalidValue;
    if (c.pro3) return (c.bn == 256) ? ig_launch_t<128, 256, 2, 4, 3, IG_PRO>(a, c.slots, st)
                                     : ig_launch_t<256, 128, 4, 2, 3, IG_PRO>(a, c.slots, st);
    return (c.bn == 128) ? ig_launch_t<128, 128, 2, 2, 2, IG_PRO>(a, c.slots, st) : ig_launch_t<128, 64, 2, 2, 2, IG_PRO>(a, c.slots, st);
  }
#define PF_IG(BMV, BNV, WMV, WNV, NSV) (bwd ? ig_launch_t<BMV, BNV, WMV, WNV, NSV, IG_BWD>(a, c.slots, st) : ig_launch_t<BMV, BNV, WMV, WNV, NSV, IG_PLAIN>(a, c.slots, st))
  if (c.bm == 256 && c.bn == 128) return PF_IG(256, 128, 4, 2, 3);
  if (c.bm == 128 && c.bn == 128) return PF_IG(128, 128, 2, 2, 2);
  if (c.bm == 256 && c.bn == 64) return PF_IG(256, 64, 4, 1, 2);
  return PF_IG(128, 64, 2, 2, 2);
#undef PF_IG
}

extern "C" int pf_conv2d_stats_groups_geom(int imgs, int H, int Wd, int C, int N, int th, int tw, int stride, int pad_h,
                                           int pad_w, int Ho, int Wo) {
  if (pf_conv3x3_c64_geom(H, Wd, C, N, th, tw, stride, pad_h, pad_w, Ho, Wo) && (imgs * Ho * Wo) % (Ho * Wo) == 0)
    return pf_conv3x3_c64_stats_groups(imgs * Ho * Wo);
  return pf_igemm_stats_groups_geom(imgs * Ho * Wo, N, 0, th * tw, C);
}

static int conv2d_fwd_launch(const void* X, const void* W, void* Y, const void* zero, const void* R, float* partial,
                             const void* bn_x, const float* bn_scale_shift, const float* bn_mean_invstd, int bn_act,
                             int imgs, int H, int Wd, int C, int N, int th, int tw, int stride, int pad_h, int pad_w,
                             int Ho, int Wo, void* stream, const float* out_scale_shift, int out_act) {
  if (out_scale_shift != nullptr && (R != nullptr || partial != nullptr || bn_x != nullptr)) return (int)hipErrorInvalidValue;
  if (imgs <= 0 || H <= 0 || Wd <= 0 || Ho <= 0 || Wo <= 0 || C <= 0 || N <= 0 || (C % 64) || (N % 8) || th < 1 || tw < 1 ||
      stride < 1)
    return (int)hipErrorInvalidValue;
  if (!pf_aligned16(X) || !pf_aligned16(W) || !pf_aligned16(Y) || !pf_aligned16(zero) || zero == nullptr ||
      (R && !pf_aligned16(R)) || (bn_x && !pf_aligned16(bn_x)))
    return (int)hipErrorInvalidValue;
  if (bn_x != nullptr && (R != nullptr || partial == nullptr || bn_scale_shift == nullptr || bn_mean_invstd == nullptr))
    return (int)hipErrorInvalidValue;
  if ((int64_t)imgs * H * Wd * C >= ((int64_t)1 << 30) || (int64_t)N * th * tw * C >= ((int64_t)1 << 30) || th * tw > 32)
    return (int)hipErrorInvalidValue;
  IgArgs a;
  a.X = (const bf16_t*)X; a.W = (const bf16_t*)W; a.Y = (bf16_t*)Y; a.zero = (const bf16_t*)zero;
  a.R = (const bf16_t*)R; a.partial = partial; a.bx = (const bf16_t*)bn_x; a.bss = bn_scale_shift; a.bmi = bn_mean_invstd;
  a.b_lo = (bn_act == PF_ACT_NONE) ? -INFINITY : 0.0f;
  a.b_hi = (bn_act == PF_ACT_RELU6) ? 6.0f : INFINITY;
  a.ss = nullptr; a.slot = nullptr; a.kq = 255.f; a.act_lo = -INFINITY; a.act_hi = INFINITY;
  a.M = imgs * Ho * Wo; a.N = N; a.C = C; a.th = th; a.tw = tw;
  a.H = H; a.Wd = Wd; a.Ho = Ho; a.Wo = Wo; a.stride = stride; a.pad_h = pad_h; a.pad_w = pad_w;
  a.x_bytes = (uint32_t)((int64_t)imgs * H * Wd * C * 2);
  a.w_bytes = (uint32_t)((int64_t)N * th * tw * C * 2);
  a.w_r0 = 0; a.w_rs = 1; a.w_s0 = 0; a.w_ss = 1; a.w_S = tw; a.w_taps_full = th * tw;
  a.o_sub = 0; a.o_y = 0; a.o_x = 0; a.o_H = 0; a.o_W = 0;
  a.oss = out_scale_shift; a.oact = out_act;
  return ig_launch(a, (hipStream_t)stream);
}

extern "C" int pf_conv2d_fwd(const void* X, const void* W, void* Y, const void* zero, const void* R, float* partial,
                             const void* bn_x, const float* bn_scale_shift, const float* bn_mean_invstd, int bn_act,
                             int imgs, int H, int Wd, int C, int N, int th, int tw, int stride, int pad_h, int pad_w,
                             int Ho, int Wo, void* stream) {
  return conv2d_fwd_launch(X, W, Y, zero, R, partial, bn_x, bn_scale_shift, bn_mean_invstd, bn_act, imgs, H, Wd, C, N, th, tw,
                           stride, pad_h, pad_w, Ho, Wo, stream, nullptr, PF_ACT_NONE);
}

#ifdef PF_IG_CODES
extern "C" int pf_probe_conv2d_fwd_codes(const void* Xc, float alpha, const void* W, void* Y, const void* zero, int imgs, int H,
                                         int Wd, int C, int N, int th, int tw, int stride, int pad_h, int pad_w, int Ho, int Wo,
                                         void* stream) {
  if ((C % 64) || (N % 64) || !pf_aligned16(Xc) || !pf_aligned16(W) || !pf_aligned16(Y)) return (int)hipErrorInvalidValue;
  IgArgs a;
  a.X = (const bf16_t*)Xc; a.W = (const bf16_t*)W; a.Y = (bf16_t*)Y; a.zero = (const bf16_t*)zero;
  a.R = nullptr; a.partial = nullptr; a.bx = nullptr; a.bss = nullptr; a.bmi = nullptr;
  a.b_lo = -INFINITY; a.b_hi = INFINITY;
  a.ss = nullptr; a.slot = nullptr; a.kq = alpha; a.act_lo = -INFINITY; a.act_hi = INFINITY;
  a.M = imgs * Ho * Wo; a.N = N; a.C = C; a.th = th; a.tw = tw;
  a.H = H; a.Wd = Wd; a.Ho = Ho; a.Wo = Wo; a.stride = stride; a.pad_h = pad_h; a.pad_w = pad_w;
  a.x_bytes = (uint32_t)((int64_t)imgs * H * Wd * C);
  a.w_bytes = (uint32_t)((int64_t)N * th * tw * C * 2);
  a.w_r0 = 0; a.w_rs = 1; a.w_s0 = 0; a.w_ss = 1; a.w_S = tw; a.w_taps_full = th * tw;
  a.o_sub = 0; a.o_y = 0; a.o_x = 0; a.o_H = 0; a.o_W = 0;
  a.oss = nullptr; a.oact = PF_ACT_NONE;
  const IgCfg c = ig_pick(a.M, a.N, false);
  if (c.bm == 256 && c.bn == 128) return ig_launch_t<256, 128, 4, 2, 3, IG_PLAIN>(a, c.slots, (hipStream_t)stream);
  if (c.bm == 128 && c.bn == 128) return ig_launch_t<128, 128, 2, 2, 2, IG_PLAIN>(a, c.slots, (hipStream_t)stream);
  if (c.bm == 256 && c.bn == 64) return ig_launch_t<256, 64, 4, 1, 2, IG_PLAIN>(a, c.slots, (hipStream_t)stream);
  return ig_launch_t<128, 64, 2, 2, 2, IG_PLAIN>(a, c.slots, (hipStream_t)stream);
}
#endif

extern "C" int pf_conv2d_fwd_affine(const void* X, const void* W, void* Y, const void* zero, const float* out_scale_shift,
                                    int out_act, int imgs, int H, int Wd, int C, int N, int th, int tw, int stride, int pad_h,
                                    int pad_w, int Ho, int Wo, void* stream) {
  if (out_scale_shift == nullptr) return (int)hipErrorInvalidValue;
  return conv2d_fwd_launch(X, W, Y, zero, nullptr, nullptr, nullptr, nullptr, nullptr, PF_ACT_NONE, imgs, H, Wd, C, N, th, tw,
                           stride, pad_h, pad_w, Ho, Wo, stream, out_scale_shift, out_act);
}

static int strided_class_groups(int imgs, int H, int Wd, int C, int stride) {
  const int bn = (C % 128 == 0) ? 128 : 64;
  int G;
  ig_grid(512, (imgs * (H / stride) * (Wd / stride) + 127) / 128, (C + bn - 1) / bn, &G);
  return G;
}

extern "C" int pf_conv2d_bwd_data_strided_stats_groups(int imgs, int H, int Wd, int C, int stride) {
  if (imgs <= 0 || H <= 0 || Wd <= 0 || C <= 0 || stride < 2 || (H % stride) || (Wd % stride)) return 0;
  return stride * stride * strided_class_groups(imgs, H, Wd, C, stride);
}

static int strided_launch(const void* dY, const void* Wt, void* dX, const void* zero, int imgs, int H, int Wd, int C, int N, int R,
                          int S, int stride, int pad_h, int pad_w, int Ho, int Wo, void* stream, float* partial, const void* bn_x,
                          const float* bss, const float* bmi, int bn_act) {
  if (imgs <= 0 || H <= 0 || Wd <= 0 || Ho <= 0 || Wo <= 0 || C <= 0 || N <= 0 || (N % 64) || (C % 8) || stride < 2 || R < stride ||
      S < stride || (H % stride) || (Wd % stride) || pad_h < 0 || pad_w < 0 || R * S > 32)
    return (int)hipErrorInvalidValue;
  if (!pf_aligned16(dY) || !pf_aligned16(Wt) || !pf_aligned16(dX) || zero == nullptr) return (int)hipErrorInvalidValue;
  if ((int64_t)imgs * Ho * Wo * N >= ((int64_t)1 << 30) || (int64_t)C * R * S * N >= ((int64_t)1 << 30)) return (int)hipErrorInvalidValue;
  const int Hc = H / stride, Wc = Wd / stride;
  for (int ay = 0; ay < stride; ++ay) {
    for (int ax = 0; ax < stride; ++ax) {
      const int r1 = (ay + pad_h) % stride, s1 = (ax + pad_w) % stride;
      const int th = (R - r1 + stride - 1) / stride, tw = (S - s1 + stride - 1) / stride;
      const int dmin_h = (ay + pad_h - r1) / stride - (th - 1), dmin_w = (ax + pad_w - s1) / stride - (tw - 1);
      IgArgs a;
      a.X = (const bf16_t*)dY; a.W = (const bf16_t*)Wt; a.Y = (bf16_t*)dX; a.zero = (const bf16_t*)zero;
      a.R = nullptr; a.partial = nullptr; a.bx = nullptr; a.bss = nullptr; a.bmi = nullptr; a.b_lo = -INFINITY; a.b_hi = INFINITY;
      if (bn_x != nullptr) {
        a.partial = partial + (int64_t)(ay * stride + ax) * strided_class_groups(imgs, H, Wd, C, stride) * 2 * C;
        a.bx = (const bf16_t*)bn_x; a.bss = bss; a.bmi = bmi;
        a.b_lo = (bn_act == PF_ACT_NONE) ? -INFINITY : 0.0f;
        a.b_hi = (bn_act == PF_ACT_RELU6) ? 6.0f : INFINITY;
      }
      a.ss = nullptr; a.slot = nullptr; a.kq = 255.f; a.act_lo = -INFINITY; a.act_hi = INFINITY;
      a.M = imgs * Hc * Wc; a.N = C; a.C = N; a.th = th; a.tw = tw;
      a.H = Ho; a.Wd = Wo; a.Ho = Hc; a.Wo = Wc; a.stride = 1; a.pad_h = -dmin_h; a.pad_w = -dmin_w;
      a.x_bytes = (uint32_t)((int64_t)imgs * Ho * Wo * N * 2);
      a.w_bytes = (uint32_t)((int64_t)C * R * S * N * 2);
      a.w_r0 = (R - 1 - r1) - (th - 1) * stride; a.w_rs = stride;
      a.w_s0 = (S - 1 - s1) - (tw - 1) * stride; a.w_ss = stride;
      a.w_S = S; a.w_taps_full = R * S;
      a.o_sub = stride; a.o_y = ay; a.o_x = ax; a.o_H = H; a.o_W = Wd; a.oss = nullptr; a.oact = PF_ACT_NONE;
      int rc;
      if (bn_x != nullptr)
        rc = (C % 128 == 0) ? ig_launch_t<128, 128, 2, 2, 2, IG_BWD, true>(a, 512, (hipStream_t)stream)
                            : ig_launch_t<128, 64, 2, 2, 2, IG_BWD, true>(a, 512, (hipStream_t)stream);
      else
        rc = (C % 128 == 0) ? ig_launch_t<128, 128, 2, 2, 2, IG_PLAIN, true>(a, 512, (hipStream_t)stream)
                            : ig_launch_t<128, 64, 2, 2, 2, IG_PLAIN, true>(a, 512, (hipStream_t)stream);
      if (rc != 0) return rc;
    }
  }
  return 0;
}

extern "C" int pf_conv2d_bwd_data_strided(const void* dY, const void* Wt, void* dX, const void* zero, int imgs, int H, int Wd,
                                          int C, int N, int R, int S, int stride, int pad_h, int pad_w, int Ho, int Wo, void* stream) {
  return strided_launch(dY, Wt, dX, zero, imgs, H, Wd, C, N, R, S, stride, pad_h, pad_w, Ho, Wo, stream, nullptr, nullptr, nullptr,
                        nullptr, PF_ACT_NONE);
}

extern "C" int pf_conv2d_bwd_data_strided_bnstats(const void* dY, const void* Wt, void* dX, const void* zero, const void* bn_x,
                                                  const float* bn_scale_shift, const float* bn_mean_invstd, int bn_act,
                                                  float* partial, int imgs, int H, int Wd, int C, int N, int R, int S, int stride,
                                                  int pad_h, int pad_w, int Ho, int Wo, void* stream) {
  if (bn_x == nullptr || partial == nullptr || bn_scale_shift == nullptr || bn_mean_invstd == nullptr || !pf_aligned16(bn_x))
    return (int)hipErrorInvalidValue;
  return strided_launch(dY, Wt, dX, zero, imgs, H, Wd, C, N, R, S, stride, pad_h, pad_w, Ho, Wo, stream, partial, bn_x,
                        bn_scale_shift, bn_mean_invstd, bn_act);
}

int pf_igemm_conv1x1(const void* X, const void* W, void* Y, const void* R, float* partial, const void* bn_x,
                     const float* bss, const float* bmi, float b_lo, float b_hi, const float* scale_shift,
                     const uint32_t* slot, float kq, float act_lo, float act_hi, int M, int N, int K, int Ho, int Wo,
                     int H, int Wd, int stride, const float* oss, int oact, hipStream_t st, int ymap) {
  int64_t rows_in = M;
  if (stride > 1 && !ymap) rows_in = (int64_t)(M / (Ho * Wo)) * H * Wd;
  if ((K % 64) || rows_in * K >= ((int64_t)1 << 30) || (int64_t)N * K >= ((int64_t)1 << 30)) return -1;
  IgArgs a;
  a.X = (const bf16_t*)X; a.W = (const bf16_t*)W; a.Y = (bf16_t*)Y; a.zero = (const bf16_t*)X;
#ifdef PF_IG_TIMING
  a.zero = (const bf16_t*)(uintptr_t)strtoull(getenv("PF_IG_TIMING_PTR"), nullptr, 0);
#endif
  a.R = (const bf16_t*)R; a.partial = partial; a.bx = (const bf16_t*)bn_x; a.bss = bss; a.bmi = bmi;
  a.b_lo = b_lo; a.b_hi = b_hi;
  a.ss = scale_shift; a.slot = slot; a.kq = kq; a.act_lo = act_lo; a.act_hi = act_hi;
  a.M = M; a.N = N; a.C = K; a.th = 1; a.tw = 1;
  if (ymap) { a.H = Ho; a.Wd = Wo; a.Ho = Ho; a.Wo = Wo; a.stride = 1; }
  else if (stride > 1) { a.H = H; a.Wd = Wd; a.Ho = Ho; a.Wo = Wo; a.stride = stride; }
  else { a.H = 1; a.Wd = 1; a.Ho = 1; a.Wo = 1; a.stride = 1; }
  a.pad_h = 0; a.pad_w = 0;
  a.x_bytes = (uint32_t)(rows_in * K * 2);
  a.w_bytes = (uint32_t)((int64_t)N * K * 2);
  a.w_r0 = 0; a.w_rs = 1; a.w_s0 = 0; a.w_ss = 1; a.w_S = 1; a.w_taps_full = 1;
  a.o_sub = 0; a.o_y = 0; a.o_x = 0; a.o_H = 0; a.o_W = 0;
  a.oss = oss; a.oact = oact;
  if (ymap) {
    if ((int64_t)(M / (Ho * Wo)) * H * Wd * N >= ((int64_t)1 << 30)) return -1;
    a.o_sub = stride; a.o_y = 0; a.o_x = 0; a.o_H = H; a.o_W = Wd;
    return (N % 128 == 0) ? ig_launch_t<128, 128, 2, 2, 2, IG_PLAIN, true>(a, 512, st) : ig_launch_t<128, 64, 2, 2, 2, IG_PLAIN, true>(a, 512, st);
  }
  return ig_launch(a, st);
}
```

### pocketflow_amd/graph.py

```python
from __future__ import annotations

import contextlib
import math
import os
import weakref
import threading
from dataclasses import dataclass, field
from typing import Callable, Dict, List, Optional, Sequence, Tuple

import numpy as np
import torch
import torch.nn.functional as F

from pocketflow_amd import hip
from pocketflow_amd.hip import check_gather
from pocketflow_amd.plan import WeightDesc
from pocketflow_amd.profiling import region

ALIGN = 64
FUSE_BN_BWD_STATS = os.environ.get('PF_FUSE_BN_BWD_STATS', '1') != '0'


def _align(n: int) -> int:
  return (n + ALIGN - 1) // ALIGN * ALIGN
# ... 496 lines not shown
      hip.bn_act_quant_apply(x, q, rows, C, scale_shift, layer.act, slot, bits if quantize else 8, quantize)
    ctx.save_for_backward(x, scale_shift, mean_invstd)
    ctx.meta = (layer.act, graph, rows, C)
    ctx.params = (gamma, beta)
    ctx.box = box
    if box is not None:
      box.update(x=x, scale_shift=scale_shift, mean_invstd=mean_invstd, act=layer.act, n_consumers=0, bwd_stats=None)
    return q

  @staticmethod
  def backward(ctx, dq):
    x, scale_shift, mean_invstd = ctx.saved_tensors
    act, graph, rows, C = ctx.meta
    pre = None
    bs = ctx.box.get('bwd_stats') if ctx.box is not None else None
    if bs is not None and bs[2] == dq.data_ptr():
      pre = bs[:2]
    dx, dgamma, dbeta = _bn_backward(dq, x, scale_shift, mean_invstd, act, graph, rows, C, params=ctx.params, pre=pre)
    return dx, dgamma, dbeta, None, None, None, None, None, None, None


class _BnEvalAct(torch.autograd.Function):

  @staticmethod
  def forward(ctx, x, gamma, beta, layer, graph):
    x = _nhwc(x)
    C = gamma.numel()
    rows = x.numel() // C
    ss = torch.empty((2, C), dtype=torch.float32, device=x.device)
    hip.bn_eval_scale_shift(gamma.detach(), beta.detach(), layer.moving_mean.tensor, layer.moving_var.tensor,
                            layer.eps, ss)
    mi = torch.stack([layer.moving_mean.tensor.float(),
                      torch.rsqrt(layer.moving_var.tensor.float() + layer.eps)]).contiguous()
    q = torch.empty_like(x)
    hip.bn_act_quant_apply(x, q, rows, C, ss, layer.act, None, 8, False)
    ctx.save_for_backward(x, ss, mi)
    ctx.meta = (layer.act, graph, rows, C)
    ctx.params = (gamma, beta)
    return q

  @staticmethod
  def backward(ctx, dq):
    x, ss, mi = ctx.saved_tensors
    act, graph, rows, C = ctx.meta
    dx, dgamma, dbeta = _bn_backward(dq, x, ss, mi, act, graph, rows, C, params=ctx.params, frozen=True)
    return dx, dgamma, dbeta, None, None


class _ActQuant(torch.autograd.Function):

  @staticmethod
  def forward(ctx, u, act, slot, bits):
    u = _nhwc(u)
    y = torch.empty_like(u)
    hip.minmax_tensor(u, slot, act)
    hip.uq_apply(u, y, slot, bits, act)
    ctx.save_for_backward(u)
    ctx.act = act
    return y

  @staticmethod
  def backward(ctx, g):
    (u,) = ctx.saved_tensors
    g = _nhwc(g)
    if g.dtype != u.dtype:
      g = g.to(u.dtype)
    dx = torch.empty_like(u)
    hip.act_grad(g, u, dx, ctx.act)
    return dx, None, None, None



class LazyAct(object):

  def __init__(self, x, scale_shift, act, slot, bits, rows, C, mean_invstd=None):
    self.x, self.scale_shift, self.act, self.slot, self.bits = x, scale_shift, act, slot, bits
    self.rows, self.C = rows, C
    self.mean_invstd = mean_invstd
    self.n_consumers = 0
    self.bwd_stats = None
    self.n_grad_consumers = 0
    self.pending = None
    self.join_ok = False
    self._q = None

  @property
  def shape(self):
    return self.x.shape

  @property
  def dtype(self):
    return self.x.dtype

  @property
  def device(self):
    return self.x.device

  def materialize(self) -> torch.Tensor:
    self.n_consumers += 2
    if self._q is None:
      self._q = _Materialize.apply(self.x, self)
    return self._q


def materialize(x):
  return x.materialize() if isinstance(x, LazyAct) else x


class _Materialize(torch.autograd.Function):
  @staticmethod
  def forward(ctx, x, lazy):
    q = torch.empty_like(x)
    quant = lazy.bits is not None
    hip.bn_act_quant_apply(x, q, lazy.rows, lazy.C, lazy.scale_shift, lazy.act, lazy.slot if quant else None,
                           lazy.bits if quant else 8, quant)
    return q

  @staticmethod
  def backward(ctx, dq):
    return dq, None


def _bn_statistics(x, rows, C, graph, st=None):
  if st is not None:
    partial, nblk = st
    return partial, nblk, graph.zero_row(C)
  nblk = _bn_blocks(rows, C)
  partial = graph.scratch(nblk * 4 * C)
  with region('bn_stats', float(x.numel() * x.element_size())):
    hip.bn_stats(x, rows, C, partial, nblk)
  return partial, nblk, x


class _BnLazy(torch.autograd.Function):

  @staticmethod
  def forward(ctx, x, gamma, beta, layer, graph, slot, bits, box, stats):
    C = gamma.numel()
    rows = x.numel() // C
    partial, nblk, piv = _bn_statistics(x, rows, C, graph, stats)
    scale_shift = torch.empty((2, C), dtype=torch.float32, device=x.device)
    mean_invstd = torch.empty((2, C), dtype=torch.float32, device=x.device)
    hip.bn_finalize(partial, nblk, rows, C, piv, gamma, beta, layer.moving_mean.tensor, layer.moving_var.tensor,
                    layer.momentum, layer.eps, True, layer.act, scale_shift, mean_invstd,
                    slot if bits is not None else None)
    ctx.save_for_backward(x, scale_shift, mean_invstd)
    ctx.meta = (layer.act, graph, rows, C)
    ctx.params = (gamma, beta)
    ctx.box = box
    ctx.set_materialize_grads(False)
    box.append(scale_shift)
    box.append(mean_invstd)
    return x.view_as(x), x.view_as(x)

  @staticmethod
  def backward(ctx, dq, dskip):
    x, scale_shift, mean_invstd = ctx.saved_tensors
    act, graph, rows, C = ctx.meta
    if dq is None:
      return dskip, None, None, None, None, None, None, None, None
    pre = None
    lazy = ctx.box[2]() if len(ctx.box) > 2 else None
    if lazy is not None and lazy.bwd_stats is not None and lazy.bwd_stats[2] == dq.data_ptr():
      pre = lazy.bwd_stats[:2]
    dx, dgamma, dbeta = _bn_backward(dq, x, scale_shift, mean_invstd, act, graph, rows, C, addend=dskip,
                                     params=ctx.params, pre=pre)
# ... 63 lines not shown
  return wk


def _out_size(size: int, k: int, stride: int, pad_total: int) -> int:
  return (size + pad_total - k) // stride + 1


def _apply_with_stats(fn, *args):
  box = []
  y = fn.apply(*args, box)
  if box[0] is not None:
    y._pf_stats = box[0]
  return y


def _conv1x1_geom(x_shape, stride):
  n, _, h, w = x_shape
  if stride == 1:
    return n * h * w, None, (h, w)
  ho, wo = -(-h // stride), -(-w // stride)
  return n * ho * wo, (ho, wo, h, w, stride), (ho, wo)


def _run_conv1x1(x, w2d, lazy, residual, want_stats, stride, out_bn=None):
  N, K = w2d.shape
  M, geom, (ho, wo) = _conv1x1_geom(x.shape, stride)
  y = torch.empty((x.shape[0], N, ho, wo), dtype=x.dtype, device=x.device, memory_format=torch.channels_last)
  if out_bn is not None:
    with region('conv1x1_fwd', float((M * K + M * N) * 2)):
      hip.conv1x1_fwd(x, w2d, y, M, N, K, scale_shift=lazy.scale_shift if lazy is not None else None,
                      act=lazy.act if lazy is not None else None, geom=geom, out_scale_shift=out_bn._eval_scale_shift(y),
                      out_act=out_bn.act)
    y._pf_bn_done = out_bn
    return y
  partial, G = None, 0
  if want_stats:
    G = hip.conv1x1_stats_groups(M, N, K, prologue=lazy is not None)
    partial = torch.empty((G, 4, N), dtype=torch.float32, device=x.device)
  ss = lazy.scale_shift if lazy is not None else None
  quant = lazy is not None and lazy.bits is not None
  nbytes = float((M * K + M * N * (2 if residual is not None else 1)) * 2)
  with region('conv1x1_fwd', nbytes):
    hip.conv1x1_fwd(x, w2d, y, M, N, K, R=residual, scale_shift=ss, act=lazy.act if lazy is not None else None,
                    slot=lazy.slot if quant else None, bits=lazy.bits if quant else 8, partial=partial, geom=geom)
  if want_stats:
    y._pf_stats = (partial, G)
  return y


class _FusedConv1x1(torch.autograd.Function):

  @staticmethod
  def forward(ctx, x, w, residual, lazy, want_stats, stride, graph, w_var, box):
    w2d = w.detach().permute(0, 2, 3, 1).reshape(w.shape[0], w.shape[1])
    res = _nhwc(residual) if residual is not None else None
    y = _run_conv1x1(x, w2d, lazy, res, want_stats, stride)
    ctx.save_for_backward(x, w2d)
    ctx.meta = (lazy, stride, graph, residual is not None, w.shape)
    ctx.w_leaf = w
    ctx.w_var = w_var
    box.append(getattr(y, '_pf_stats', None))
    return y

  @staticmethod
  def backward(ctx, dy):
    x, w2d = ctx.saved_tensors
    lazy, stride, graph, has_res, w_shape = ctx.meta
    dy = _nhwc(dy)
    N, K = w2d.shape
    M, geom, _ = _conv1x1_geom(x.shape, stride)
    ss = lazy.scale_shift if lazy is not None else None
    quant = lazy is not None and lazy.bits is not None
    act = lazy.act if lazy is not None else None
    dx = dw = None
    if ctx.needs_input_grad[1]:
      S = hip.conv1x1_wrw_splits(M, N, K)

      def wrw(dwk, scratch):
        hip.conv1x1_wrw(dy, x, dwk.view(N, K), scratch((S + 32) * N * K), M, N, K, scale_shift=ss, act=act,
                        slot=lazy.slot if quant else None, bits=lazy.bits if quant else 8, geom=geom)
      dw = _filter_grad(graph, ctx.w_leaf, ctx.w_var, (dy, x, w2d, ss, lazy), 'conv1x1_wrw', float((M * K + M * N) * 2), wrw)
    if ctx.needs_input_grad[0]:
      wt = _bwd_data_weight(graph, ctx.w_var, ctx.w_leaf).view(K, N)
      if geom is None:
        dx = torch.empty_like(x)
      else:
        dx = torch.zeros_like(x)
      fuse_stats = (FUSE_BN_BWD_STATS and lazy is not None and lazy.n_consumers == 1 and geom is None
                    and lazy.mean_invstd is not None and lazy.act in ('Relu', 'Relu6'))
      join = (JOIN_TWO_CONSUMERS and lazy is not None and lazy.join_ok and lazy.n_consumers == 2
              and lazy.n_grad_consumers == 2)
      second = join and lazy.pending is not None
      res = lazy.pending if (second and geom is None) else None
      with region('conv1x1_bwd_data', float((M * K * (2 if (fuse_stats or res is not None) else 1) + M * N) * 2)):
        if fuse_stats:
          G = hip.conv1x1_stats_groups(M, K, N)
          partial = torch.empty((G, 2, K), dtype=torch.float32, device=x.device)
          hip.conv1x1_bwd_data_bnstats(dy, wt, dx, x, lazy.scale_shift, lazy.mean_invstd, lazy.act, partial, M, N, K)
          lazy.bwd_stats = (partial, G, dx.data_ptr())
        elif res is not None:
          hip.conv1x1_fwd(dy, wt, dx, M, K, N, R=res)
        else:
          hip.conv1x1_fwd(dy, wt, dx, M, K, N, geom=geom, ymap=geom is not None)
      if join:
        if not second:
          lazy.pending, dx = dx, None
        else:
          if res is None:
            dx = dx + lazy.pending
          lazy.pending = None
    return dx, dw, (dy if has_res else None), None, None, None, None, None, None


JOIN_TWO_CONSUMERS = os.environ.get('PF_JOIN_TWO_CONSUMERS', '1') != '0'
USE_SEG_TRANSPOSE = os.environ.get('PF_SEG_TRANSPOSE', '1') != '0'
OWN_POOL = os.environ.get('PF_OWN_POOL', '1') != '0'
OWN_CONV2D_WRW = os.environ.get('PF_OWN_CONV2D_WRW', '1') != '0'
OWN_CONV2D_WRW_MIN_C = int(os.environ.get('PF_OWN_CONV2D_WRW_MIN_C', '64'))
OWN_CONV2D_BWD_STRIDED = os.environ.get('PF_OWN_CONV2D_BWD_STRIDED', '1') != '0'
OWN_CONV2D = os.environ.get('PF_OWN_CONV2D', '1') != '0'
OWN_STEM = os.environ.get('PF_OWN_STEM', '1') != '0'
OWN_DEPTHWISE = os.environ.get('PF_OWN_DEPTHWISE', '1') != '0'
OWN_CONV_IM2COL = os.environ.get('PF_OWN_CONV_IM2COL', '1') != '0'
CONVG_BF16_NARROW = os.environ.get('PF_CONVG_BF16_NARROW', '0') != '0'
FOLD_EVAL_BN = os.environ.get('PF_FOLD_EVAL_BN', '1') != '0'
OWN_CONV_GENERIC = os.environ.get('PF_OWN_CONV_GENERIC', '1') != '0'
DEPTHWISE_ANY_DEVICE = False


def _run_conv2d(x, w_krsc, stride, pad, want_stats, out_bn=None):
  B, C, H, W = x.shape
  N, R, S, _ = w_krsc.shape
  Ho, Wo = _out_size(H, R, stride, 2 * pad[0]), _out_size(W, S, stride, 2 * pad[1])
  y = torch.empty((B, N, Ho, Wo), dtype=x.dtype, device=x.device, memory_format=torch.channels_last)
  M = B * Ho * Wo
  if out_bn is not None:
    with region('conv2d_fwd', float((B * H * W * C + M * N) * 2)):
      hip.conv2d_fwd(x, w_krsc, y, B, H, W, C, N, R, S, stride, pad[0], pad[1], Ho, Wo,
                     out_scale_shift=out_bn._eval_scale_shift(y), out_act=out_bn.act)
    y._pf_bn_done = out_bn
    return y
  partial, G = None, 0
  if want_stats:
    G = hip.conv2d_stats_groups(M, N, geom=(B, H, W, C, N, R, S, stride, pad[0], pad[1], Ho, Wo))
    partial = torch.empty((G, 4, N), dtype=torch.float32, device=x.device)
  with region('conv2d_fwd', float((B * H * W * C + M * N) * 2)):
    hip.conv2d_fwd(x, w_krsc, y, B, H, W, C, N, R, S, stride, pad[0], pad[1], Ho, Wo, partial=partial)
  if want_stats:
    y._pf_stats = (partial, G)
  return y


class _Conv2dIgemm(torch.autograd.Function):

  @staticmethod
  def forward(ctx, x, w, stride, pad, want_stats, graph, bn_box, w_var, box):
    ctx.w_var = w_var
    w_krsc = w.detach().permute(0, 2, 3, 1)
    y = _run_conv2d(x, w_krsc, stride, pad, want_stats)
    ctx.save_for_backward(x, w)
    ctx.meta = (stride, pad, graph, bn_box)
    box.append(getattr(y, '_pf_stats', None))
    return y

  @staticmethod
  def backward(ctx, dy):
    x, w = ctx.saved_tensors
    stride, pad, graph, bn_box = ctx.meta
    dy = _nhwc(dy)
    dx = dw = None
    N, C, R, S = w.shape
    B, _, H, W = x.shape
    Ho, Wo = dy.shape[2], dy.shape[3]
    if ctx.needs_input_grad[1]:
      splits = hip.conv2d_wrw_splits(B * Ho * Wo, N, C, R * S) if (OWN_CONV2D_WRW and C >= OWN_CONV2D_WRW_MIN_C) else 0
      nbytes = float((x.numel() + dy.numel()) * 2)
      if splits > 0:
        def wrw(dwk, scratch):
          hip.conv2d_wrw(dy, x, dwk, scratch((splits + 32) * N * R * S * C), B, H, W, C, N, R, S, stride, pad[0], pad[1], Ho, Wo)
        dw = _filter_grad(graph, w, ctx.w_var, (dy, x), 'conv2d_wrw', nbytes, wrw)
      elif OWN_CONV2D_WRW and OWN_CONV_GENERIC and x.is_cuda and dy.dtype == x.dtype and w.dtype == x.dtype:
        gs = hip.convg_wrw_splits(B, C, N, R, S, Ho, Wo)
        dwk = torch.empty((N, R, S, C), dtype=w.dtype, device=x.device)
        with region('conv2d_wrw', nbytes):
          hip.convg_wrw(dy, x, dwk, graph.scratch(gs * N * R * S * C), B, H, W, C, N, R, S, stride, pad[0], pad[1], Ho, Wo)
        dw = dwk.permute(0, 3, 1, 2)
      else:
        with region('conv2d_wrw', nbytes):
          dw = torch.ops.aten.convolution_backward(dy, x, w.detach(), None, [stride, stride], list(pad), [1, 1], False,
                                                   [0, 0], 1, [False, True, False])[1]
    if ctx.needs_input_grad[0]:
      mfma = N % 64 == 0 and C % 8 == 0 and igemm_limits_ok(dy.numel(), w.numel(), R * S)
      by_classes = (OWN_CONV2D_BWD_STRIDED and stride > 1 and H % stride == 0 and W % stride == 0 and R >= stride and S >= stride
                    and dy.dtype == torch.bfloat16)
      if mfma and (stride == 1 or by_classes):
        wb = _bwd_data_weight(graph, ctx.w_var, w)
        dx = torch.empty_like(x)
# ... 253 lines not shown
def fused_conv1x1_ok(x, conv) -> bool:
  t = x.x if isinstance(x, LazyAct) else x
  return (conv.k == 1 and conv.bias is None and fusable_tensor(t) and t.dim() == 4
          and conv.kernel.ref_shape[2] % 8 == 0 and conv.kernel.ref_shape[3] % 8 == 0
          and conv.padding in ('SAME', 'VALID', 0) and conv.graph.fuse_conv1x1)



def _same_pads(size: int, k: int, stride: int) -> Tuple[int, int]:
  out = -(-size // stride)
  total = max((out - 1) * stride + k - size, 0)
  return total // 2, total - total // 2


def _symmetric_pads(x: torch.Tensor, ph: Tuple[int, int], pw: Tuple[int, int]):
  if ph[0] == ph[1] and pw[0] == pw[1]:
    return x, (ph[0], pw[0])
  return F.pad(x, (pw[0], pw[1], ph[0], ph[1])), (0, 0)


def variance_scaling_init(ref_shape, fan_in: int):
  std = math.sqrt(1.0 / max(1.0, fan_in)) / .87962566103423978

  def init(rng: np.random.RandomState):
    from scipy.stats import truncnorm
    return truncnorm.rvs(-2, 2, size=ref_shape, random_state=rng).astype(np.float32) * np.float32(std)
  return init


def glorot_uniform_init(ref_shape, fan_in: int, fan_out: int):
  limit = math.sqrt(6.0 / (fan_in + fan_out))
  return lambda rng: rng.uniform(-limit, limit, size=ref_shape).astype(np.float32)


def truncated_normal_init(ref_shape, stddev: float):
  def init(rng: np.random.RandomState):
    from scipy.stats import truncnorm
    return truncnorm.rvs(-2, 2, size=ref_shape, random_state=rng).astype(np.float32) * np.float32(stddev)
  return init


def constant_init(ref_shape, value: float):
  return lambda rng: np.full(ref_shape, value, dtype=np.float32)


GATHER_MAX_CIN = 8192


def gather_pays(k: int, cin: int, kept: int, cout: int, dtype) -> bool:
  return False


class Conv2D:

  def __init__(self, graph: Graph, name: str, cin: int, cout: int, k: int, stride: int = 1,
               padding: str = 'SAME', use_bias: bool = False, kernel_name: str = 'kernel',
               bias_name: str = 'bias', init=None, l2: bool = True):
    self.graph, self.k, self.stride, self.padding = graph, k, stride, padding
    ref_shape = (k, k, cin, cout)
    init = init or variance_scaling_init(ref_shape, k * k * cin)
    self.kernel = graph.store.add(name + '/' + kernel_name, ref_shape, 'conv', True, l2, init)
    self.bias = (graph.store.add(name + '/' + bias_name, (cout,), 'bias', True, l2, constant_init((cout,), 0.0))
                 if use_bias else None)
    self.op = graph.add_matmul_op('Conv2D', name + '/Conv2D', self.kernel)

  def __call__(self, x, residual: Optional[torch.Tensor] = None, want_stats: bool = False, out_bn=None) -> torch.Tensor:
    w = self.kernel.tensor
    if out_bn is not None and (residual is not None or not out_bn.folds_into_producer()):
      out_bn = None
    if self.graph.taps is not None:
      return _tapped(self, materialize(x), residual)
    if self.kernel.gather_host is not None:
      return self._call_gathered(x, residual, out_bn)
    if fused_conv1x1_ok(x, self):
      lazy = x if isinstance(x, LazyAct) else None
      if lazy is not None:
        lazy.n_consumers += 1
      elif getattr(x, '_pf_bn', None) is not None:
        x._pf_bn['n_consumers'] += 2
      xin = lazy.x if lazy is not None else _nhwc(x)
      if torch.is_grad_enabled() and (xin.requires_grad or w.requires_grad):
        if lazy is not None and xin.requires_grad:
          lazy.n_grad_consumers += 1
        return _apply_with_stats(_FusedConv1x1, xin, w, residual, lazy, want_stats, self.stride, self.graph, self.kernel)
      w2d = w.detach().permute(0, 2, 3, 1).reshape(w.shape[0], w.shape[1])
      return _run_conv1x1(xin, w2d, lazy, _nhwc(residual) if residual is not None else None, want_stats,
                          self.stride, out_bn=out_bn)
    x = materialize(x)
    b = self.bias.tensor.to(x.dtype) if self.bias is not None else None
    ph, pw, out_hw = self._geometry(x)
    if (self.padding == 'SAME' and residual is None and x.shape[1] == 3 and self.k == 3 and self.stride == 2
        and own_stem3_ok(x, self, (ph[0], pw[0]), out_hw)):
      if torch.is_grad_enabled() and w.requires_grad:
        return _Stem3Conv.apply(x, w, self.graph, self.kernel, (ph[0], pw[0]), out_hw)
      return _run_stem3(x, w, (ph[0], pw[0]), out_hw)
    x, pad = _symmetric_pads(x, ph, pw)
    if residual is None and own_stem_ok(x, self, pad):
      if torch.is_grad_enabled() and (x.requires_grad or w.requires_grad):
        return _StemConv.apply(x, w, self.graph, self.kernel)
      return _run_stem(x, w)
    if own_conv2d_ok(x, self, pad):
      bn_box = getattr(x, '_pf_bn', None)
      if bn_box is not None:
        bn_box['n_consumers'] += 1
      xin = _nhwc(x)
      if torch.is_grad_enabled() and (xin.requires_grad or w.requires_grad):
        y = _apply_with_stats(_Conv2dIgemm, xin, w, self.stride, pad, want_stats, self.graph, bn_box, self.kernel)
      else:
        y = _run_conv2d(xin, w.detach().permute(0, 2, 3, 1), self.stride, pad, want_stats, out_bn=out_bn)
      return y if residual is None else y + residual
    bn_box = getattr(x, '_pf_bn', None)
    if bn_box is not None:
      bn_box['n_consumers'] += 2
    if im2col_conv_ok(x, self, pad):
      y = _ConvIm2col.apply(_nhwc(x), w, self.stride, pad, out_hw, self.graph, self.kernel)
    elif convg_ok(x, w):
      y = conv_generic(x, w, self.bias.tensor if self.bias is not None else None, self.stride, pad, out_hw, self.graph)
    else:
      y = F.conv2d(x, w, b, stride=self.stride, padding=pad)
    return y if residual is None else y + residual

  def _geometry(self, x):
    ph = pw = (0, 0)
    if isinstance(self.padding, int):
      ph = pw = (self.padding, self.padding)
    elif self.padding == 'SAME' and self.k > 1:
      ph = _same_pads(x.shape[2], self.k, self.stride)
      pw = _same_pads(x.shape[3], self.k, self.stride)
    return ph, pw, (_out_size(x.shape[2], self.k, self.stride, ph[0] + ph[1]),
                    _out_size(x.shape[3], self.k, self.stride, pw[0] + pw[1]))

  def _call_gathered(self, x, residual, out_bn) -> torch.Tensor:
    var = self.kernel
    w = var.tensor
    x = materialize(x)
    if torch.is_grad_enabled() and (w.requires_grad or x.requires_grad):
      raise RuntimeError('%s: a shrunk (channel-gathered) convolution runs in inference only: call it under torch.no_grad() '
                         'on a graph finalised with requires_grad=False' % var.name)
    if x.dim() != 4 or x.shape[1] != var.cin_full:
      raise ValueError('%s: input of shape %s, the layer has %d input channels' % (var.name, tuple(x.shape), var.cin_full))
    ph, pw, (Ho, Wo) = self._geometry(x)
    x, pad = _symmetric_pads(x, ph, pw)
    x = _nhwc(x)
    B, C, H, Wd = x.shape
    N = w.shape[0]
    wk = _krsc(w, x.dtype)
    y = torch.empty((B, N, Ho, Wo), dtype=x.dtype, device=x.device, memory_format=torch.channels_last)
    bias = None if self.bias is None else self.bias.tensor.detach().float().contiguous()
    res = None if residual is None else _nhwc(residual).to(x.dtype)
    ss = out_bn._eval_scale_shift(y) if out_bn is not None else None
    with region('conv_gather_fwd', float((x.numel() + y.numel() * (2 if res is not None else 1)) * x.element_size())):
      hip.conv_gather_fwd(x, wk, var.gather, y, B, H, Wd, C, N, self.k, self.k, self.stride, pad[0], pad[1], Ho, Wo,
                          bias=bias, residual=res, scale_shift=ss, act=out_bn.act if out_bn is not None else None)
    if out_bn is not None:
      y._pf_bn_done = out_bn
    return y

  def plain(self, x: torch.Tensor) -> torch.Tensor:
    taps, self.graph.taps = self.graph.taps, None
    fuse, self.graph.fuse_conv1x1 = self.graph.fuse_conv1x1, False
    try:
      return self(x)
    finally:
      self.graph.taps, self.graph.fuse_conv1x1 = taps, fuse


# ... 301 lines not shown
```

### pocketflow_amd/hip.py

```python
from __future__ import annotations

import ctypes
import os
from ctypes import c_float, c_int, c_int64, c_void_p

import numpy as np
import torch

_LIB_PATH = os.environ.get('PF_HIP_LIB') or os.path.join(os.path.dirname(os.path.abspath(__file__)), 'csrc', 'libpocketflow_hip.so')

PF_F32, PF_BF16 = 0, 1
PF_ACT_NONE, PF_ACT_RELU, PF_ACT_RELU6 = 0, 1, 2
PF_BUCKET_TENSOR, PF_BUCKET_CHANNEL, PF_BUCKET_SPLIT = 0, 1, 2
PF_CHUNK = 4096

SEG_DTYPE = np.dtype([('offset', '<i8'), ('len', '<i8'), ('RS', '<i4'), ('layout', '<i4'),
                      ('I', '<i4'), ('O', '<i4'), ('mode', '<i4'), ('bits', '<i4'),
                      ('bucket_size', '<i4'), ('n_bucket', '<i4'), ('slot_offset', '<i8'),
                      ('cb_offset', '<i8')])
BLOCK_DTYPE = np.dtype([('seg', '<i4'), ('chunk', '<i4'), ('row0', '<i4'), ('nrows', '<i4')])
assert SEG_DTYPE.itemsize == 64 and BLOCK_DTYPE.itemsize == 16

ACT_CODES = {None: PF_ACT_NONE, 'none': PF_ACT_NONE, 'Relu': PF_ACT_RELU, 'relu': PF_ACT_RELU,
             'Relu6': PF_ACT_RELU6, 'relu6': PF_ACT_RELU6}

SYMBOLS = [
    'pf_error_string', 'pf_version', 'pf_minmax_slots_init', 'pf_minmax_tensor', 'pf_minmax_decode',
    'pf_uq_apply', 'pf_act_grad', 'pf_seg_minmax', 'pf_seg_uq_apply', 'pf_seg_nuq_apply',
    'pf_seg_nuq_codebook_grad', 'pf_seg_normalize', 'pf_ws_bkup_merge_abs', 'pf_kth_largest_nonneg',
    'pf_ws_mask_apply', 'pf_count_nonzero', 'pf_cp_build_mask', 'pf_cp_mask_grad', 'pf_adam_flat',
    'pf_momentum_flat', 'pf_ce_distill_fwd_bwd', 'pf_bn_stats', 'pf_bn_finalize',
    'pf_bn_act_quant_apply', 'pf_bn_bwd_stats', 'pf_bn_bwd_finalize', 'pf_bn_bwd_apply', 'pf_bn_bwd_apply_add',
    'pf_bn_eval_scale_shift',
    'pf_conv1x1_stats_groups', 'pf_conv1x1_stats_groups_k', 'pf_conv1x1_fwd', 'pf_conv1x1_bwd_data_bnstats', 'pf_conv1x1_wrw_splits',
    'pf_conv1x1_wrw', 'pf_conv2d_stats_groups', 'pf_conv2d_fwd', 'pf_conv2d_wrw_splits', 'pf_conv2d_wrw', 'pf_maxpool_fwd', 'pf_maxpool_bwd', 'pf_seg_transpose', 'pf_conv_stem_supported', 'pf_conv_stem_fwd', 'pf_conv_stem_wrw_slabs', 'pf_conv_stem_wrw',
    'pf_image_resize_bilinear', 'pf_depthwise_supported', 'pf_depthwise_groups', 'pf_depthwise_fwd', 'pf_depthwise_bwd_data',
    'pf_depthwise_wrw', 'pf_conv2d_stats_groups_geom', 'pf_tuning_reload',
    'pf_adam_flat_dev', 'pf_momentum_flat_dev', 'pf_set_floats',
    'pf_convg_fwd', 'pf_convg_bwd_data', 'pf_convg_small_splits', 'pf_convg_wrw_splits', 'pf_convg_wrw', 'pf_conv2d_bwd_data_strided',
    'pf_prox_groups', 'pf_prox_norms', 'pf_prox_apply', 'pf_im2col', 'pf_col2im',
    'pf_conv_stem3_supported', 'pf_conv_stem3_fwd', 'pf_conv_stem3_wrw_slabs', 'pf_conv_stem3_wrw',
    'pf_conv1x1_fwd_affine', 'pf_conv2d_fwd_affine', 'pf_conv2d_bwd_data_strided_stats_groups',
    'pf_conv2d_bwd_data_strided_bnstats',
    'pf_cpr_gather', 'pf_cpr_gram_ws', 'pf_cpr_gram', 'pf_cpr_ista', 'pf_cpr_lstsq_splits', 'pf_cpr_lstsq_step', 'pf_cpr_lstsq_resid',
    'pf_conv_gather_fwd',
]


class HipLibraryMissing(RuntimeError):
  pass


def lib_path() -> str:
  return _LIB_PATH


def _load() -> ctypes.CDLL:
  if not os.path.exists(_LIB_PATH):
    raise HipLibraryMissing(
        'pocketflow_amd: %s not found -- build it with `python -c "import __graft_entry__ as g; '
        'g.build()"` or pocketflow_amd/csrc/build.sh.  There is no CPU fallback.' % _LIB_PATH)
  lib = ctypes.CDLL(_LIB_PATH)
  lib.pf_error_string.restype = ctypes.c_char_p
  lib.pf_error_string.argtypes = [c_int]
  lib.pf_version.restype = c_int
  for name in SYMBOLS:
    fn = getattr(lib, name)
    if name not in ('pf_error_string',):
      fn.restype = c_int
  lib.pf_cpr_gram_ws.restype = c_int64
  return lib


_lib = _load()


def _check(err: int, what: str) -> None:
  if err != 0:
    raise RuntimeError('%s failed: hipError %d (%s)' % (what, err, _lib.pf_error_string(err).decode()))


_raw_stream = getattr(torch._C, '_cuda_getCurrentRawStream', None)
_get_device = getattr(torch._C, '_cuda_getDevice', None)


def _stream() -> c_void_p:
  if _raw_stream is not None and _get_device is not None:
    return c_void_p(_raw_stream(_get_device()))
  return c_void_p(torch.cuda.current_stream().cuda_stream)


def _ptr(t) -> c_void_p:
  if t is None:
    return c_void_p(0)
  return c_void_p(t.data_ptr())


def dtype_code(t: torch.Tensor) -> int:
  if t.dtype == torch.float32:
    return PF_F32
  if t.dtype == torch.bfloat16:
    return PF_BF16
  raise TypeError('unsupported dtype %s (float32 / bfloat16 only)' % t.dtype)


def _dev(t: torch.Tensor) -> None:
  if not t.is_cuda:
    raise RuntimeError('pocketflow_amd kernels run on the GPU only (got a %s tensor)' % t.device)


def version() -> int:
  return int(_lib.pf_version())


def tuning_reload() -> None:
  _check(_lib.pf_tuning_reload(), 'pf_tuning_reload')



def minmax_slots_init(slots: torch.Tensor) -> None:
  _dev(slots)
  _check(_lib.pf_minmax_slots_init(_ptr(slots), c_int64(slots.numel() // 2), _stream()), 'pf_minmax_slots_init')


def minmax_tensor(x: torch.Tensor, slot: torch.Tensor, act=None) -> None:
  _dev(x)
  _check(_lib.pf_minmax_tensor(_ptr(x), c_int64(x.numel()), c_int(dtype_code(x)), c_int(ACT_CODES[act]),
                               _ptr(slot), _stream()), 'pf_minmax_tensor')
# ... 241 lines not shown
  _check(_lib.pf_bn_stats(_ptr(x), c_int(dtype_code(x)), c_int64(rows), c_int(C), _ptr(partial), c_int(n_blocks),
                          _stream()), 'pf_bn_stats')


def bn_finalize(partial, n_blocks, rows, C, x, gamma, beta, moving_mean, moving_var, momentum, eps,
                training: bool, act, scale_shift, mean_invstd, slot) -> None:
  _check(_lib.pf_bn_finalize(_ptr(partial), c_int(n_blocks), c_int64(rows), c_int(C), _ptr(x),
                             c_int(dtype_code(x)), _ptr(gamma), _ptr(beta), _ptr(moving_mean), _ptr(moving_var),
                             c_float(momentum), c_float(eps), c_int(1 if training else 0), c_int(ACT_CODES[act]),
                             _ptr(scale_shift), _ptr(mean_invstd), _ptr(slot), _stream()), 'pf_bn_finalize')


def bn_act_quant_apply(x, q, rows, C, scale_shift, act, slot, bits: int, quantize: bool) -> None:
  _check(_lib.pf_bn_act_quant_apply(_ptr(x), _ptr(q), c_int(dtype_code(x)), c_int64(rows), c_int(C),
                                    _ptr(scale_shift), c_int(ACT_CODES[act]), _ptr(slot), c_int(int(bits)),
                                    c_int(1 if quantize else 0), _stream()), 'pf_bn_act_quant_apply')


def bn_bwd_stats(dq, x, rows, C, scale_shift, mean_invstd, act, partial, n_blocks) -> None:
  _check(_lib.pf_bn_bwd_stats(_ptr(dq), _ptr(x), c_int(dtype_code(x)), c_int64(rows), c_int(C), _ptr(scale_shift),
                              _ptr(mean_invstd), c_int(ACT_CODES[act]), _ptr(partial), c_int(n_blocks),
                              _stream()), 'pf_bn_bwd_stats')


def bn_bwd_finalize(partial, n_blocks, C, dgamma, dbeta) -> None:
  _check(_lib.pf_bn_bwd_finalize(_ptr(partial), c_int(n_blocks), c_int(C), _ptr(dgamma), _ptr(dbeta), _stream()),
         'pf_bn_bwd_finalize')


def bn_bwd_apply(dq, x, dx, rows, C, scale_shift, mean_invstd, dgamma, dbeta, act, addend=None) -> None:
  _check(_lib.pf_bn_bwd_apply_add(_ptr(dq), _ptr(x), _ptr(addend), _ptr(dx), c_int(dtype_code(x)), c_int64(rows),
                                  c_int(C), _ptr(scale_shift), _ptr(mean_invstd), _ptr(dgamma), _ptr(dbeta),
                                  c_int(ACT_CODES[act]), _stream()), 'pf_bn_bwd_apply_add')


def bn_eval_scale_shift(gamma, beta, moving_mean, moving_var, eps: float, scale_shift) -> None:
  _check(_lib.pf_bn_eval_scale_shift(_ptr(gamma), _ptr(beta), _ptr(moving_mean), _ptr(moving_var), c_float(eps),
                                     c_int(gamma.numel()), _ptr(scale_shift), _stream()), 'pf_bn_eval_scale_shift')



def conv1x1_stats_groups(M: int, N: int, K: int, prologue: bool = False) -> int:
  return int(_lib.pf_conv1x1_stats_groups_k(c_int(M), c_int(N), c_int(K), c_int(1 if prologue else 0)))


def conv1x1_wrw_splits(M: int, N: int, K: int) -> int:
  return int(_lib.pf_conv1x1_wrw_splits(c_int(M), c_int(N), c_int(K)))


def conv1x1_fwd(X, W, Y, M: int, N: int, K: int, R=None, scale_shift=None, act=None, slot=None, bits: int = 8,
                partial=None, geom=None, ymap: bool = False, out_scale_shift=None, out_act=None) -> None:
  _dev(X)
  Ho, Wo, H, Wd, stride = geom if geom is not None else (0, 0, 0, 0, 1)
  if out_scale_shift is not None:
    if R is not None or partial is not None or slot is not None or ymap:
      raise ValueError('the folded output pass takes no residual, statistics, quantiser or row map')
    _check(_lib.pf_conv1x1_fwd_affine(_ptr(X), _ptr(W), _ptr(Y), _ptr(scale_shift), c_int(ACT_CODES[act]), _ptr(out_scale_shift),
                                      c_int(ACT_CODES[out_act]), c_int(M), c_int(N), c_int(K), c_int(Ho), c_int(Wo), c_int(H),
                                      c_int(Wd), c_int(stride), _stream()), 'pf_conv1x1_fwd_affine')
    return
  _check(_lib.pf_conv1x1_fwd(_ptr(X), _ptr(W), _ptr(Y), _ptr(R), _ptr(scale_shift), c_int(ACT_CODES[act]),
                             _ptr(slot), c_int(int(bits)), _ptr(partial), c_int(M), c_int(N), c_int(K), c_int(Ho),
                             c_int(Wo), c_int(H), c_int(Wd), c_int(stride), c_int(1 if ymap else 0), _stream()),
         'pf_conv1x1_fwd')


def conv1x1_wrw(dY, X, dW, workspace, M: int, N: int, K: int, scale_shift=None, act=None, slot=None,
                bits: int = 8, geom=None) -> None:
  _dev(X)
  Ho, Wo, H, Wd, stride = geom if geom is not None else (0, 0, 0, 0, 1)
  _check(_lib.pf_conv1x1_wrw(_ptr(dY), _ptr(X), _ptr(dW), c_int(dtype_code(dW)), _ptr(workspace), _ptr(scale_shift),
                             c_int(ACT_CODES[act]), _ptr(slot), c_int(int(bits)), c_int(M), c_int(N), c_int(K),
                             c_int(Ho), c_int(Wo), c_int(H), c_int(Wd), c_int(stride), _stream()), 'pf_conv1x1_wrw')


def conv1x1_bwd_data_bnstats(dY, Wt, dQ, bn_x, bn_scale_shift, bn_mean_invstd, bn_act, partial, M: int, N: int,
                             K: int) -> None:
  _dev(dY)
  _check(_lib.pf_conv1x1_bwd_data_bnstats(_ptr(dY), _ptr(Wt), _ptr(dQ), _ptr(bn_x), _ptr(bn_scale_shift),
                                          _ptr(bn_mean_invstd), c_int(ACT_CODES[bn_act]), _ptr(partial), c_int(M),
                                          c_int(N), c_int(K), _stream()), 'pf_conv1x1_bwd_data_bnstats')



_zero_page = {}


def zero_page(device):
  key = str(device)
  z = _zero_page.get(key)
  if z is None:
    z = _zero_page[key] = torch.zeros(256, dtype=torch.bfloat16, device=device)
  return z


def conv2d_stats_groups(M: int, N: int, geom=None) -> int:
  if geom is None:
    raise ValueError('conv2d_stats_groups: pass geom = (imgs, H, Wd, C, N, th, tw, stride, pad_h, pad_w, Ho, Wo) of the pf_conv2d_fwd call')
  return int(_lib.pf_conv2d_stats_groups_geom(*[c_int(int(v)) for v in geom]))


def conv2d_fwd(X, W, Y, imgs: int, H: int, Wd: int, C: int, N: int, th: int, tw: int, stride: int, pad_h: int,
               pad_w: int, Ho: int, Wo: int, R=None, partial=None, bn_x=None, bn_scale_shift=None,
               bn_mean_invstd=None, bn_act=None, out_scale_shift=None, out_act=None) -> None:
  _dev(X)
  if out_scale_shift is not None:
    if R is not None or partial is not None or bn_x is not None:
      raise ValueError('the folded output pass takes no residual or statistics')
    _check(_lib.pf_conv2d_fwd_affine(_ptr(X), _ptr(W), _ptr(Y), _ptr(zero_page(X.device)), _ptr(out_scale_shift),
                                     c_int(ACT_CODES[out_act]), c_int(imgs), c_int(H), c_int(Wd), c_int(C), c_int(N), c_int(th),
                                     c_int(tw), c_int(stride), c_int(pad_h), c_int(pad_w), c_int(Ho), c_int(Wo), _stream()),
           'pf_conv2d_fwd_affine')
    return
  _check(_lib.pf_conv2d_fwd(_ptr(X), _ptr(W), _ptr(Y), _ptr(zero_page(X.device)), _ptr(R), _ptr(partial), _ptr(bn_x),
                            _ptr(bn_scale_shift), _ptr(bn_mean_invstd), c_int(ACT_CODES[bn_act]), c_int(imgs), c_int(H),
                            c_int(Wd), c_int(C), c_int(N), c_int(th), c_int(tw), c_int(stride), c_int(pad_h),
                            c_int(pad_w), c_int(Ho), c_int(Wo), _stream()), 'pf_conv2d_fwd')


def conv2d_wrw_splits(M: int, N: int, C: int, taps: int) -> int:
  return int(_lib.pf_conv2d_wrw_splits(c_int(M), c_int(N), c_int(C), c_int(taps)))


def conv2d_wrw(dY, X, dW, workspace, imgs: int, H: int, Wd: int, C: int, N: int, th: int, tw: int, stride: int,
               pad_h: int, pad_w: int, Ho: int, Wo: int) -> None:
  _dev(X)
  _check(_lib.pf_conv2d_wrw(_ptr(dY), _ptr(X), _ptr(dW), c_int(dtype_code(dW)), _ptr(workspace), c_int(imgs), c_int(H),
                            c_int(Wd), c_int(C), c_int(N), c_int(th), c_int(tw), c_int(stride), c_int(pad_h),
                            c_int(pad_w), c_int(Ho), c_int(Wo), _stream()), 'pf_conv2d_wrw')


def depthwise_supported(C: int, k: int, stride: int) -> bool:
  return bool(_lib.pf_depthwise_supported(c_int(C), c_int(k), c_int(stride)))


def depthwise_groups(B: int, Ho: int, Wo: int, C: int) -> int:
  return int(_lib.pf_depthwise_groups(c_int(B), c_int(Ho), c_int(Wo), c_int(C)))


def depthwise_fwd(X, W, Y, B: int, H: int, Wd: int, C: int, k: int, stride: int, pad_h: int, pad_w: int, Ho: int, Wo: int,
                  partial=None) -> None:
  _dev(X)
  _check(_lib.pf_depthwise_fwd(_ptr(X), _ptr(W), _ptr(Y), c_int(dtype_code(X)), _ptr(partial), c_int(B), c_int(H), c_int(Wd),
                               c_int(C), c_int(k), c_int(stride), c_int(pad_h), c_int(pad_w), c_int(Ho), c_int(Wo),
                               _stream()), 'pf_depthwise_fwd')


def depthwise_bwd_data(dY, W, dX, B: int, H: int, Wd: int, C: int, k: int, stride: int, pad_h: int, pad_w: int, Ho: int,
                       Wo: int) -> None:
  _dev(dY)
  _check(_lib.pf_depthwise_bwd_data(_ptr(dY), _ptr(W), _ptr(dX), c_int(dtype_code(dY)), c_int(B), c_int(H), c_int(Wd), c_int(C),
                                    c_int(k), c_int(stride), c_int(pad_h), c_int(pad_w), c_int(Ho), c_int(Wo), _stream()),
         'pf_depthwise_bwd_data')


def depthwise_wrw(dY, X, dW, slabs, B: int, H: int, Wd: int, C: int, k: int, stride: int, pad_h: int, pad_w: int, Ho: int,
                  Wo: int) -> None:
  _dev(X)
  if slabs.dtype != torch.float32 or slabs.numel() < (depthwise_groups(B, Ho, Wo, C) + 32) * C * k * k:
    raise TypeError('depthwise_wrw: float32 workspace of (groups + 32) * C * k * k elements')
  _check(_lib.pf_depthwise_wrw(_ptr(dY), _ptr(X), _ptr(dW), c_int(dtype_code(X)), c_int(dtype_code(dW)), _ptr(slabs), c_int(B),
                               c_int(H), c_int(Wd), c_int(C), c_int(k), c_int(stride), c_int(pad_h), c_int(pad_w), c_int(Ho),
                               c_int(Wo), _stream()), 'pf_depthwise_wrw')


def conv2d_bwd_data_strided_stats_groups(B: int, H: int, Wd: int, C: int, stride: int) -> int:
# ... 189 lines not shown
```

Baseline: 11370.

## Fuse projection-shortcut gradient join into 1x1 bwd-data GEMM with strided residual map

When a BN output feeds both a strided projection 1x1 conv and the main branch, the first backward-data result is now computed compactly (no zero-filled scatter) and kept pending. The second consumer's bwd-data GEMM then adds it in the epilogue through a strided row map, optionally fusing BN backward stats. This removes a zeros_like allocation, a separate elementwise add and a full-tensor read/write. The cost is new kernel template variants (stream and igemm) with extra residual loads and index math, plus more planning logic that may limit which shapes qualify.

```diff
diff --git a/include/pocketflow_hip.h b/include/pocketflow_hip.h
--- a/include/pocketflow_hip.h
+++ b/include/pocketflow_hip.h
@@ -123,6 +123,10 @@
 int pf_conv1x1_bwd_data_bnstats(const void* dY, const void* Wt, void* dQ, const void* bn_x,
                                 const float* bn_scale_shift, const float* bn_mean_invstd, int bn_act,
                                 float* partial, int M, int N, int K, void* stream);
+int pf_conv1x1_join_plan(int M, int N, int K, int with_stats);
+int pf_conv1x1_bwd_data_join(const void* dY, const void* Wt, void* dQ, const void* R, int r_Ho, int r_Wo, int r_H, int r_W,
+                             int r_stride, const void* bn_x, const float* bn_scale_shift, const float* bn_mean_invstd,
+                             int bn_act, float* partial, int M, int N, int K, void* stream);
 int pf_conv1x1_wrw_splits(int M, int N, int K);
 int pf_conv1x1_wrw(const void* dY, const void* X, void* dW, int dw_dtype, float* workspace,
                    const float* scale_shift, int act, const uint32_t* slot, int bits, int M, int N,
diff --git a/pocketflow_amd/csrc/pf_conv.hip b/pocketflow_amd/csrc/pf_conv.hip
--- a/pocketflow_amd/csrc/pf_conv.hip
+++ b/pocketflow_amd/csrc/pf_conv.hip
@@ -271,6 +271,7 @@
 int pf_conv_stream_plan(int M, int N, int K, int* nw_out);
 int pf_conv_stream_groups(int nsplit);
 int pf_conv_stream_launch(const ConvArgs& a, bool pro, bool bwd, hipStream_t st);
+bool pf_conv_stream_join_ok(int nw, bool with_stats);
 
 extern "C" int pf_conv1x1_stats_groups(int M, int N) {
   const int bn = conv_bn_of(N);
@@ -284,7 +285,8 @@
 int pf_igemm_conv1x1(const void* X, const void* W, void* Y, const void* R, float* partial, const void* bn_x,
                      const float* bss, const float* bmi, float b_lo, float b_hi, const float* scale_shift,
                      const uint32_t* slot, float kq, float act_lo, float act_hi, int M, int N, int K, int Ho, int Wo,
-                     int H, int Wd, int stride, const float* oss, int oact, hipStream_t st, int ymap = 0);
+                     int H, int Wd, int stride, const float* oss, int oact, hipStream_t st, int ymap = 0, const int* rgeom = nullptr);
+bool pf_igemm_join_ok(int M, int N, int K);
 #ifndef PF_CONV_IGEMM_PLAIN_MINK
 #define PF_CONV_IGEMM_PLAIN_MINK 256
 #endif
@@ -301,11 +303,26 @@
   return pf_conv1x1_stats_groups(M, N);
 }
 
+static int conv_join_kernel(int M, int N, int K, bool with_stats) {
+  if (M <= 0 || N <= 0 || K <= 0) return 0;
+  int nw = 0;
+  if (pf_conv_stream_plan(M, K, N, &nw) > 0) return pf_conv_stream_join_ok(nw, with_stats) ? 1 : 0;
+  if (conv_use_igemm(false, N) && pf_igemm_join_ok(M, K, N)) return 2;
+  return 0;
+}
+
+#define PF_JOIN_STATS_IGEMM_MIN_M (1 << 17)
+extern "C" int pf_conv1x1_join_plan(int M, int N, int K, int with_stats) {
+  const int k = conv_join_kernel(M, N, K, with_stats != 0);
+  if (k == 2 && with_stats && M < PF_JOIN_STATS_IGEMM_MIN_M) return 0;
+  return k;
+}
+
 static int conv_fwd_launch(const void* X, const void* W, void* Y, const void* R, const float* scale_shift,
                            int act, const uint32_t* slot, int bits, float* partial, int M, int N, int K,
                            int Ho, int Wo, int H, int Wd, int stride, int ymap, const void* bx,
                            const float* bss, const float* bmi, int bact, void* stream, const float* oss = nullptr,
-                           int oact = PF_ACT_NONE) {
+                           int oact = PF_ACT_NONE, const int* rgeom = nullptr) {
   if (oss != nullptr && (R != nullptr || partial != nullptr || bx != nullptr || ymap)) return (int)hipErrorInvalidValue;
   if (M <= 0 || N <= 0 || K <= 0 || (K % 8) || (N % 8)) return (int)hipErrorInvalidValue;
   if (!pf_aligned16(X) || !pf_aligned16(W) || !pf_aligned16(Y) || (R && !pf_aligned16(R)))
@@ -325,7 +342,9 @@
   a.b_lo = (bact == PF_ACT_NONE) ? -INFINITY : 0.0f;
   a.b_hi = (bact == PF_ACT_RELU6) ? 6.0f : INFINITY;
   a.oss = oss; a.oact = oact;
-  if (bx != nullptr && (R != nullptr || partial == nullptr || bss == nullptr || bmi == nullptr || stride != 1 ||
+  a.rHo = 0; a.rWo = 0; a.rH = 0; a.rW = 0; a.rstride = 1;
+  if (rgeom != nullptr) { a.rHo = rgeom[0]; a.rWo = rgeom[1]; a.rH = rgeom[2]; a.rW = rgeom[3]; a.rstride = rgeom[4]; }
+  if (bx != nullptr && ((R != nullptr && rgeom == nullptr) || partial == nullptr || bss == nullptr || bmi == nullptr || stride != 1 ||
                         !pf_aligned16(bx)))
     return (int)hipErrorInvalidValue;
   const int bn = conv_bn_of(N);
@@ -335,6 +354,15 @@
   hipStream_t st = (hipStream_t)stream;
   const bool pro = scale_shift != nullptr;
   if (bx != nullptr && pro) return (int)hipErrorInvalidValue;
+  if (rgeom != nullptr) {
+    if (pro || ymap || stride != 1 || oss != nullptr || R == nullptr) return (int)hipErrorInvalidValue;
+    const int plan = conv_join_kernel(M, K, N, bx != nullptr);
+    int r = -1;
+    if (plan == 1) r = pf_conv_stream_launch(a, false, bx != nullptr, st);
+    else if (plan == 2) r = pf_igemm_conv1x1(X, W, Y, R, partial, bx, bss, bmi, a.b_lo, a.b_hi, nullptr, nullptr, a.kq, a.act_lo,
+                                             a.act_hi, M, N, K, 0, 0, 0, 0, 1, nullptr, PF_ACT_NONE, st, 0, rgeom);
+    return (r >= 0) ? r : (int)hipErrorInvalidValue;
+  }
   {
     const int r = pf_conv_stream_launch(a, pro, bx != nullptr, st);
     if (r >= 0) return r;
@@ -391,6 +419,20 @@
                                            float* partial, int M, int N, int K, void* stream) {
   return conv_fwd_launch(dY, Wt, dQ, nullptr, nullptr, PF_ACT_NONE, nullptr, 8, partial, M, K, N, 0, 0, 0, 0, 1, 0,
                          bn_x, bn_scale_shift, bn_mean_invstd, bn_act, stream);
+}
+
+extern "C" int pf_conv1x1_bwd_data_join(const void* dY, const void* Wt, void* dQ, const void* R, int r_Ho, int r_Wo, int r_H, int r_W,
+                                        int r_stride, const void* bn_x, const float* bn_scale_shift, const float* bn_mean_invstd,
+                                        int bn_act, float* partial, int M, int N, int K, void* stream) {
+  if (R == nullptr || r_stride < 1) return (int)hipErrorInvalidValue;
+  if (r_stride > 1) {
+    if (r_H <= 0 || r_W <= 0 || (M % (r_H * r_W)) || r_Ho != (r_H + r_stride - 1) / r_stride || r_Wo != (r_W + r_stride - 1) / r_stride)
+      return (int)hipErrorInvalidValue;
+  }
+  if (conv_join_kernel(M, N, K, bn_x != nullptr) == 0) return (int)hipErrorInvalidValue;
+  const int rgeom[5] = {r_Ho, r_Wo, r_H, r_W, r_stride};
+  return conv_fwd_launch(dY, Wt, dQ, R, nullptr, PF_ACT_NONE, nullptr, 8, (bn_x != nullptr) ? partial : nullptr, M, K, N, 0, 0, 0, 0, 1,
+                         0, bn_x, bn_scale_shift, bn_mean_invstd, bn_act, stream, nullptr, PF_ACT_NONE, rgeom);
 }
 
 #define WR_TN 128
diff --git a/pocketflow_amd/csrc/pf_conv_common.h b/pocketflow_amd/csrc/pf_conv_common.h
--- a/pocketflow_amd/csrc/pf_conv_common.h
+++ b/pocketflow_amd/csrc/pf_conv_common.h
@@ -47,7 +47,17 @@
   float b_lo, b_hi;
   const float* oss;
   int oact;
+  int rHo, rWo, rH, rW, rstride;
 };
+
+__device__ __forceinline__ int64_t rmap_row(int m, int Ho, int Wo, int H, int W, int stride) {
+  const int hw = H * W;
+  const int img = m / hw, rem = m - img * hw;
+  const int h = rem / W, w = rem - h * W;
+  const int hq = h / stride, wq = w / stride;
+  if (hq * stride != h || wq * stride != w) return -1;
+  return ((int64_t)img * Ho + hq) * Wo + wq;
+}
 
 __device__ __forceinline__ uint4 out_affine8(const uint4& c, const float* __restrict__ oss, int N, int n, int act) {
   float f[8];
diff --git a/pocketflow_amd/csrc/pf_conv_stream.hip b/pocketflow_amd/csrc/pf_conv_stream.hip
--- a/pocketflow_amd/csrc/pf_conv_stream.hip
+++ b/pocketflow_amd/csrc/pf_conv_stream.hip
@@ -5,7 +5,7 @@
 #define ST_WAVES 8
 #define ST_GRID 256
 
-template <int NW, bool PRO, bool BWD, bool MAP, bool AFF = false>
+template <int NW, bool PRO, bool BWD, bool MAP, bool AFF = false, bool RMAP = false, bool BR = false>
 __global__ __launch_bounds__(ST_THREADS) void k_conv1x1_stream(const ConvArgs a, const int nsplit) {
   constexpr int JM = (NW == 256) ? 1 : 2;
   constexpr int RS = 16 * JM;
@@ -62,16 +62,19 @@
 
   const int wswz = (KV >= 16) ? l15 : (l15 & 7);
   const bf16_t* __restrict__ side = BWD ? a.bx : nullptr;
-  const bool has_r = !BWD && a.R != nullptr;
+  static_assert(!BR || BWD, "BR is a variant of BWD");
+  const bool has_r = BWD ? BR : (a.R != nullptr);
   const int wvec = lane % VPR, wrow = lane / VPR;
 
   f32x4 acc[NI][JM];
   uint4 ring[D][NR];
   uint4 rres[NP];
   uint2 rr[NI][JM];
-  float st_s[8], st_q[8], st_mn[8], st_mx[8];
-#pragma unroll
-  for (int j = 0; j < 8; ++j) { st_s[j] = 0.f; st_q[j] = 0.f; st_mn[j] = INFINITY; st_mx[j] = -INFINITY; }
+  float st_s[8], st_q[8], st_mn[BR ? 1 : 8], st_mx[BR ? 1 : 8];
+#pragma unroll
+  for (int j = 0; j < 8; ++j) { st_s[j] = 0.f; st_q[j] = 0.f; }
+#pragma unroll
+  for (int j = 0; j < (BR ? 1 : 8); ++j) { st_mn[j] = INFINITY; st_mx[j] = -INFINITY; }
 
   int ld_s = s_first, ld_kc = 0;
   auto issue = [&](uint4 (&r)[NR]) {
@@ -100,12 +103,17 @@
 #pragma unroll
     for (int j = 0; j < JM; ++j) {
       const int m = s * RS + j * 16 + l15;
-      const int64_t orow = (m < a.M) ? ((MAP && a.ymap) ? map_row(a, m) : (int64_t)m) : 0;
+      int64_t orow = (m < a.M) ? ((MAP && a.ymap) ? map_row(a, m) : (int64_t)m) : 0;
+      bool live = m < a.M;
+      if constexpr (RMAP) {
+        orow = live ? rmap_row(m, a.rHo, a.rWo, a.rH, a.rW, a.rstride) : -1;
+        live = orow >= 0;
+      }
 #pragma unroll
       for (int i = 0; i < NI; ++i) {
         const int n = n0 + i * 16 + q * 4;
         uint2 v = make_uint2(0, 0);
-        if (m < a.M && n < a.N) v = *reinterpret_cast<const uint2*>(a.R + orow * a.N + n);
+        if (live && n < a.N) v = *reinterpret_cast<const uint2*>(a.R + orow * a.N + n);
         rr[i][j] = v;
       }
     }
@@ -113,7 +121,8 @@
 #pragma clang loop unroll(full)
   for (int d = 0; d < D; ++d)
     if (d < T) issue(ring[d]);
-  if (has_r && cnt > 0) issue_res(s_first);
+  constexpr bool RLATE = BR && NW == 256;
+  if (has_r && !RLATE && cnt > 0) issue_res(s_first);
   if (side != nullptr && cnt > 0) {
 #pragma unroll
     for (int p = 0; p < NP; ++p) issue_side(s_first, p);
@@ -186,7 +195,32 @@
     if (++ckc == KC) { ckc = 0; cs += sstep; }
     if (!last) continue;
 
-    if (has_r) {
+    if constexpr (RLATE) {
+      const int m = s * RS + l15;
+      int64_t orow = m;
+      bool live = m < a.M;
+      if constexpr (RMAP) {
+        orow = live ? rmap_row(m, a.rHo, a.rWo, a.rH, a.rW, a.rstride) : -1;
+        live = orow >= 0;
+      }
+#pragma unroll
+      for (int ib = 0; ib < NI; ib += 8) {
+        uint2 t[8];
+#pragma unroll
+        for (int i = 0; i < 8; ++i) {
+          const int n = n0 + (ib + i) * 16 + q * 4;
+          t[i] = make_uint2(0, 0);
+          if (live && n < a.N) t[i] = *reinterpret_cast<const uint2*>(a.R + orow * a.N + n);
+        }
+#pragma unroll
+        for (int i = 0; i < 8; ++i) {
+          acc[ib + i][0][0] += __uint_as_float(t[i].x << 16); acc[ib + i][0][1] += __uint_as_float(t[i].x & 0xFFFF0000u);
+          acc[ib + i][0][2] += __uint_as_float(t[i].y << 16); acc[ib + i][0][3] += __uint_as_float(t[i].y & 0xFFFF0000u);
+        }
+        __builtin_amdgcn_sched_barrier(0);
+      }
+    }
+    if (has_r && !RLATE) {
 #pragma unroll
       for (int i = 0; i < NI; ++i)
 #pragma unroll
@@ -203,9 +237,10 @@
         *reinterpret_cast<uint2*>(Cs + (j * 16 + l15) * CS_LD + i * 16 + q * 4) = w;
       }
     const bool more = (cs < NS);
-    if (has_r && more) issue_res(cs);
+    if (has_r && !RLATE && more) issue_res(cs);
     float bpr[32];
-    if (BWD && NW != 128) {
+    constexpr bool BPL = (NW == 128) || BR;
+    if (BWD && !BPL) {
 #pragma unroll
       for (int qq = 0; qq < 4; ++qq)
 #pragma unroll
@@ -214,7 +249,7 @@
 #pragma unroll
       for (int i = 0; i < 32; ++i) bpr[i] = 0.f;
     }
-    constexpr int CB = (NW == 128) ? 1 : 4;
+    constexpr int CB = (NW == 128 || (BR && NW == 256)) ? 1 : (BR ? 2 : 4);
     uint4 cv[CB];
 #pragma unroll
     for (int p = 0; p < NP; ++p) {
@@ -230,12 +265,12 @@
       if (side != nullptr && more) issue_side(cs, p);
       if (m < a.M && n < a.N) {
         const int64_t orow = (MAP && a.ymap) ? map_row(a, m) : (int64_t)m;
-        if (BWD) {
+        if constexpr (BWD) {
           float f[8], xv[8];
           unpack8(c, f);
           unpack8(sv, xv);
-          const float* bp = (NW == 128) ? (aux + wvec * 8) : bpr;
-          constexpr int BPS = (NW == 128) ? NW : 8;
+          const float* bp = BPL ? (aux + wvec * 8) : bpr;
+          constexpr int BPS = BPL ? NW : 8;
 #pragma unroll
           for (int j = 0; j < 8; ++j) {
             const float u = fmaf(bp[j], xv[j], bp[BPS + j]);
@@ -269,8 +304,10 @@
       for (int j = 0; j < 8; ++j) {
         st_s[j] += __shfl_xor(st_s[j], o, 64);
         st_q[j] += __shfl_xor(st_q[j], o, 64);
-        st_mn[j] = fminf(st_mn[j], __shfl_xor(st_mn[j], o, 64));
-        st_mx[j] = fmaxf(st_mx[j], __shfl_xor(st_mx[j], o, 64));
+        if constexpr (!BR) {
+          st_mn[j] = fminf(st_mn[j], __shfl_xor(st_mn[j], o, 64));
+          st_mx[j] = fmaxf(st_mx[j], __shfl_xor(st_mx[j], o, 64));
+        }
       }
     }
     __syncthreads();
@@ -279,8 +316,10 @@
       for (int j = 0; j < 8; ++j) {
         red[(0 * ST_WAVES + wave) * NW + lane * 8 + j] = st_s[j];
         red[(1 * ST_WAVES + wave) * NW + lane * 8 + j] = st_q[j];
-        red[(2 * ST_WAVES + wave) * NW + lane * 8 + j] = st_mn[j];
-        red[(3 * ST_WAVES + wave) * NW + lane * 8 + j] = st_mx[j];
+        if constexpr (!BR) {
+          red[(2 * ST_WAVES + wave) * NW + lane * 8 + j] = st_mn[j];
+          red[(3 * ST_WAVES + wave) * NW + lane * 8 + j] = st_mx[j];
+        }
       }
     }
     __syncthreads();
@@ -320,13 +359,15 @@
 
 int pf_conv_stream_groups(int nsplit) { return ST_GRID / nsplit; }
 
-template <int NW, bool PRO, bool BWD, bool MAP, bool AFF = false>
+bool pf_conv_stream_join_ok(int nw, bool with_stats) { return !with_stats || nw == 64 || nw == 256; }
+
+template <int NW, bool PRO, bool BWD, bool MAP, bool AFF = false, bool RMAP = false, bool BR = false>
 static int stream_launch_t(const ConvArgs& a, int nsplit, hipStream_t st) {
   const int JM = (NW == 256) ? 1 : 2, RS = 16 * JM;
   const size_t aux_fl = PRO ? 2 * (size_t)a.K : (BWD ? 4 * (size_t)NW : 0);
   const size_t lds = (size_t)NW * a.K * 2 + aux_fl * 4 + (size_t)ST_WAVES * RS * (NW + 8) * 2;
-  if (int e = pf_require_lds(reinterpret_cast<const void*>(&k_conv1x1_stream<NW, PRO, BWD, MAP, AFF>), lds)) return e;
-  k_conv1x1_stream<NW, PRO, BWD, MAP, AFF><<<ST_GRID, ST_THREADS, lds, st>>>(a, nsplit);
+  if (int e = pf_require_lds(reinterpret_cast<const void*>(&k_conv1x1_stream<NW, PRO, BWD, MAP, AFF, RMAP, BR>), lds)) return e;
+  k_conv1x1_stream<NW, PRO, BWD, MAP, AFF, RMAP, BR><<<ST_GRID, ST_THREADS, lds, st>>>(a, nsplit);
   PF_LAUNCH_CHECK();
   return 0;
 }
@@ -336,6 +377,17 @@
   const int nsplit = pf_conv_stream_plan(a.M, a.N, a.K, &nw);
   if (nsplit == 0) return -1;
   const bool map = a.stride != 1;
+  if (a.rstride > 1 || (bwd && a.R != nullptr)) {
+    if (!pf_conv_stream_join_ok(nw, bwd) || pro || map || a.oss != nullptr || a.R == nullptr) return -1;
+    const bool rmap = a.rstride > 1;
+#define PF_STJ(NWV) do { if (!bwd) return stream_launch_t<NWV, false, false, false, false, true, false>(a, nsplit, st);         \
+                         return rmap ? stream_launch_t<NWV, false, true, false, false, true, true>(a, nsplit, st)              \
+                                     : stream_launch_t<NWV, false, true, false, false, false, true>(a, nsplit, st); } while (0)
+    if (nw == 64) PF_STJ(64);
+    if (nw == 256) PF_STJ(256);
+#undef PF_STJ
+    return stream_launch_t<128, false, false, false, false, true, false>(a, nsplit, st);
+  }
   if (a.oss != nullptr) {
     if (map || bwd) return -1;
 #define PF_STA(NWV) do { return pro ? stream_launch_t<NWV, true, false, false, true>(a, nsplit, st)     \
diff --git a/pocketflow_amd/csrc/pf_igemm.h b/pocketflow_amd/csrc/pf_igemm.h
--- a/pocketflow_amd/csrc/pf_igemm.h
+++ b/pocketflow_amd/csrc/pf_igemm.h
@@ -36,6 +36,7 @@
   int o_sub, o_y, o_x, o_H, o_W;
   const float* oss;
   int oact;
+  int rHo, rWo, rH, rW, rstride;
 };
 
 template <int N> __device__ __forceinline__ void wait_vm() { asm volatile("s_waitcnt vmcnt(%0)" ::"n"(N) : "memory"); }
diff --git a/pocketflow_amd/csrc/pf_igemm.hip b/pocketflow_amd/csrc/pf_igemm.hip
--- a/pocketflow_amd/csrc/pf_igemm.hip
+++ b/pocketflow_amd/csrc/pf_igemm.hip
@@ -34,9 +34,10 @@
 #define PF_IG_XB 2
 #endif
 
-template <int BM, int BN, int WM, int WN, int NS, int MODE, bool SUB = false, bool AFF = false>
+template <int BM, int BN, int WM, int WN, int NS, int MODE, bool SUB = false, bool AFF = false, bool RMAP = false, bool BR = false>
 __global__ __launch_bounds__(64 * WM * WN) void k_igemm(const IgArgs a) {
   constexpr bool BWD = (MODE == IG_BWD), PRO = (MODE == IG_PRO);
+  static_assert(!BR || BWD, "BR is a variant of IG_BWD");
   static_assert(!PRO || NS == 2 || NS == 3, "the in-LDS prologue pass is written for the 2- and 3-stage rings");
   constexpr bool PRO3 = PRO && NS == 3;
   constexpr int NWC = WM * WN;
@@ -179,17 +180,23 @@
 #pragma unroll
       for (int j = 0; j < JM; ++j) acc[i][j] = (f32x4){0.f, 0.f, 0.f, 0.f};
     uint2 rr[NI][JM];
-    const bool has_r = !BWD && a.R != nullptr;
+    const bool has_r = BWD ? BR : (a.R != nullptr);
     constexpr bool RPRE = BM * BN <= 128 * 256;
     auto load_residual = [&]() {
 #pragma unroll
       for (int j = 0; j < JM; ++j) {
         const int m = m0 + wm * WR + j * 16 + l15;
+        int64_t rrow = m;
+        bool live = m < a.M;
+        if constexpr (RMAP) {
+          rrow = live ? rmap_row(m, a.rHo, a.rWo, a.rH, a.rW, a.rstride) : -1;
+          live = rrow >= 0;
+        }
 #pragma unroll
         for (int i = 0; i < NI; ++i) {
           const int n = n0 + wn * WC + i * 16 + q * 4;
           rr[i][j] = make_uint2(0, 0);
-          if (m < a.M && n < a.N) rr[i][j] = *reinterpret_cast<const uint2*>(a.R + (int64_t)m * a.N + n);
+          if (live && n < a.N) rr[i][j] = *reinterpret_cast<const uint2*>(a.R + rrow * a.N + n);
         }
       }
     };
@@ -378,11 +385,17 @@
 #pragma unroll
         for (int j = 0; j < JM; ++j) {
           const int m = m0 + wm * WR + j * 16 + l15;
+          int64_t rrow = m;
+          bool live = m < a.M;
+          if constexpr (RMAP) {
+            rrow = live ? rmap_row(m, a.rHo, a.rWo, a.rH, a.rW, a.rstride) : -1;
+            live = rrow >= 0;
+          }
 #pragma unroll
           for (int i = 0; i < NI; ++i) {
             const int n = n0 + wn * WC + i * 16 + q * 4;
-            if (m < a.M && n < a.N) {
-              const uint2 r = *reinterpret_cast<const uint2*>(a.R + (int64_t)m * a.N + n);
+            if (live && n < a.N) {
+              const uint2 r = *reinterpret_cast<const uint2*>(a.R + rrow * a.N + n);
               acc[i][j][0] += __uint_as_float(r.x << 16); acc[i][j][1] += __uint_as_float(r.x & 0xFFFF0000u);
               acc[i][j][2] += __uint_as_float(r.y << 16); acc[i][j][3] += __uint_as_float(r.y & 0xFFFF0000u);
             }
@@ -439,7 +452,7 @@
     };
     constexpr bool etid = true;
     float bpr[32];
-    if (BWD) {
+    if (BWD && !BR) {
 #pragma unroll
       for (int qq = 0; qq < 4; ++qq)
 #pragma unroll
@@ -473,8 +486,8 @@
             float f[8], xv[8];
             unpack8(c, f);
             unpack8(rres[pp], xv);
-            const float* bp = bpr;
-            constexpr int BPS = 8;
+            const float* bp = BR ? (bpl + wvec * 8) : bpr;
+            constexpr int BPS = BR ? BN : 8;
 #pragma unroll
             for (int j = 0; j < 8; ++j) {
               const float u = fmaf(bp[j], xv[j], bp[BPS + j]);
@@ -589,7 +602,7 @@
 
 extern "C" int pf_conv2d_stats_groups(int M, int N) { return pf_igemm_stats_groups(M, N, 0); }
 
-template <int BM, int BN, int WM, int WN, int NS, int MODE, bool SUB = false, bool AFF = false>
+template <int BM, int BN, int WM, int WN, int NS, int MODE, bool SUB = false, bool AFF = false, bool RMAP = false, bool BR = false>
 static int ig_launch_t(IgArgs& a, int slots, hipStream_t st) {
   constexpr bool BWD = (MODE == IG_BWD), PRO3 = (MODE == IG_PRO && NS == 3);
   constexpr int THREADS = 64 * WM * WN;
@@ -601,8 +614,8 @@
   const size_t lds = base + (BWD ? 4 * BN * 4 : 0) + (PRO3 ? 2 * (size_t)a.C * 4 : 0);
   if (PRO3 && a.C > CV_MAXK) return (int)hipErrorInvalidValue;
   const size_t lds_max = base + (BWD ? 4 * BN * 4 : 0) + (PRO3 ? 2 * (size_t)CV_MAXK * 4 : 0);
-  if (int e = pf_require_lds(reinterpret_cast<const void*>(&k_igemm<BM, BN, WM, WN, NS, MODE, SUB, AFF>), lds_max)) return e;
-  k_igemm<BM, BN, WM, WN, NS, MODE, SUB, AFF><<<grid, THREADS, lds, st>>>(a);
+  if (int e = pf_require_lds(reinterpret_cast<const void*>(&k_igemm<BM, BN, WM, WN, NS, MODE, SUB, AFF, RMAP, BR>), lds_max)) return e;
+  k_igemm<BM, BN, WM, WN, NS, MODE, SUB, AFF, RMAP, BR><<<grid, THREADS, lds, st>>>(a);
   PF_LAUNCH_CHECK();
   return 0;
 }
@@ -678,6 +691,7 @@
   a.w_r0 = 0; a.w_rs = 1; a.w_s0 = 0; a.w_ss = 1; a.w_S = tw; a.w_taps_full = th * tw;
   a.o_sub = 0; a.o_y = 0; a.o_x = 0; a.o_H = 0; a.o_W = 0;
   a.oss = out_scale_shift; a.oact = out_act;
+  a.rHo = 0; a.rWo = 0; a.rH = 0; a.rW = 0; a.rstride = 1;
   return ig_launch(a, (hipStream_t)stream);
 }
 
@@ -766,6 +780,7 @@
       a.w_s0 = (S - 1 - s1) - (tw - 1) * stride; a.w_ss = stride;
       a.w_S = S; a.w_taps_full = R * S;
       a.o_sub = stride; a.o_y = ay; a.o_x = ax; a.o_H = H; a.o_W = Wd; a.oss = nullptr; a.oact = PF_ACT_NONE;
+      a.rHo = 0; a.rWo = 0; a.rH = 0; a.rW = 0; a.rstride = 1;
       int rc;
       if (bn_x != nullptr)
         rc = (C % 128 == 0) ? ig_launch_t<128, 128, 2, 2, 2, IG_BWD, true>(a, 512, (hipStream_t)stream)
@@ -795,10 +810,16 @@
                         bn_scale_shift, bn_mean_invstd, bn_act);
 }
 
+bool pf_igemm_join_ok(int M, int N, int K) {
+  if ((K % 64) || (N % 64) || (int64_t)M * K >= ((int64_t)1 << 30) || (int64_t)N * K >= ((int64_t)1 << 30)) return false;
+  const IgCfg c = ig_pick(M, N, false);
+  return c.bm == 128 && c.slots == 512 && c.bn == ((N % 128 == 0) ? 128 : 64);
+}
+
 int pf_igemm_conv1x1(const void* X, const void* W, void* Y, const void* R, float* partial, const void* bn_x,
                      const float* bss, const float* bmi, float b_lo, float b_hi, const float* scale_shift,
                      const uint32_t* slot, float kq, float act_lo, float act_hi, int M, int N, int K, int Ho, int Wo,
-                     int H, int Wd, int stride, const float* oss, int oact, hipStream_t st, int ymap) {
+                     int H, int Wd, int stride, const float* oss, int oact, hipStream_t st, int ymap, const int* rgeom) {
   int64_t rows_in = M;
   if (stride > 1 && !ymap) rows_in = (int64_t)(M / (Ho * Wo)) * H * Wd;
   if ((K % 64) || rows_in * K >= ((int64_t)1 << 30) || (int64_t)N * K >= ((int64_t)1 << 30)) return -1;
@@ -820,6 +841,19 @@
   a.w_r0 = 0; a.w_rs = 1; a.w_s0 = 0; a.w_ss = 1; a.w_S = 1; a.w_taps_full = 1;
   a.o_sub = 0; a.o_y = 0; a.o_x = 0; a.o_H = 0; a.o_W = 0;
   a.oss = oss; a.oact = oact;
+  a.rHo = 0; a.rWo = 0; a.rH = 0; a.rW = 0; a.rstride = 1;
+  if (rgeom != nullptr) {
+    if (!pf_igemm_join_ok(M, N, K) || ymap || stride != 1 || R == nullptr || scale_shift != nullptr || oss != nullptr) return -1;
+    a.rHo = rgeom[0]; a.rWo = rgeom[1]; a.rH = rgeom[2]; a.rW = rgeom[3]; a.rstride = rgeom[4];
+    const bool rmap = a.rstride > 1, bwd = bn_x != nullptr, wide = (N % 128 == 0);
+    if (!rmap && !bwd) return ig_launch(a, st);
+    if (!bwd) return wide ? ig_launch_t<128, 128, 2, 2, 2, IG_PLAIN, false, false, true, false>(a, 512, st)
+                          : ig_launch_t<128, 64, 2, 2, 2, IG_PLAIN, false, false, true, false>(a, 512, st);
+    if (rmap) return wide ? ig_launch_t<128, 128, 2, 2, 2, IG_BWD, false, false, true, true>(a, 512, st)
+                          : ig_launch_t<128, 64, 2, 2, 2, IG_BWD, false, false, true, true>(a, 512, st);
+    return wide ? ig_launch_t<128, 128, 2, 2, 2, IG_BWD, false, false, false, true>(a, 512, st)
+                : ig_launch_t<128, 64, 2, 2, 2, IG_BWD, false, false, false, true>(a, 512, st);
+  }
   if (ymap) {
     if ((int64_t)(M / (Ho * Wo)) * H * Wd * N >= ((int64_t)1 << 30)) return -1;
     a.o_sub = stride; a.o_y = 0; a.o_x = 0; a.o_H = H; a.o_W = Wd;
diff --git a/pocketflow_amd/graph.py b/pocketflow_amd/graph.py
--- a/pocketflow_amd/graph.py
+++ b/pocketflow_amd/graph.py
@@ -602,6 +602,8 @@
     self.n_grad_consumers = 0
     self.pending = None
     self.join_ok = False
+    self.pending_geom = None
+    self.dense_out = None
     self._q = None
 
   @property
@@ -831,18 +833,37 @@
       dw = _filter_grad(graph, ctx.w_leaf, ctx.w_var, (dy, x, w2d, ss, lazy), 'conv1x1_wrw', float((M * K + M * N) * 2), wrw)
     if ctx.needs_input_grad[0]:
       wt = _bwd_data_weight(graph, ctx.w_var, ctx.w_leaf).view(K, N)
-      if geom is None:
-        dx = torch.empty_like(x)
-      else:
-        dx = torch.zeros_like(x)
       fuse_stats = (FUSE_BN_BWD_STATS and lazy is not None and lazy.n_consumers == 1 and geom is None
                     and lazy.mean_invstd is not None and lazy.act in ('Relu', 'Relu6'))
       join = (JOIN_TWO_CONSUMERS and lazy is not None and lazy.join_ok and lazy.n_consumers == 2
               and lazy.n_grad_consumers == 2)
       second = join and lazy.pending is not None
       res = lazy.pending if (second and geom is None) else None
+      join_entry = getattr(hip, 'conv1x1_bwd_data_join', None) if PROJ_JOIN else None
+      compact = (join and not second and geom is not None and join_entry is not None and lazy.dense_out is not None
+                 and hip.conv1x1_join_plan(x.shape[0] * x.shape[2] * x.shape[3], lazy.dense_out, K) != 0)
+      rgeom = lazy.pending_geom if res is not None else None
+      join_stats = (res is not None and join_entry is not None and PROJ_JOIN_STATS and FUSE_BN_BWD_STATS
+                    and lazy.mean_invstd is not None and lazy.act in ('Relu', 'Relu6')
+                    and hip.conv1x1_join_plan(M, N, K, True) != 0)
+      if compact:
+        dx = torch.empty((x.shape[0], K, geom[0], geom[1]), dtype=x.dtype, device=x.device, memory_format=torch.channels_last)
+      elif geom is None:
+        dx = torch.empty_like(x)
+      else:
+        dx = torch.zeros_like(x)
       with region('conv1x1_bwd_data', float((M * K * (2 if (fuse_stats or res is not None) else 1) + M * N) * 2)):
-        if fuse_stats:
+        if compact:
+          hip.conv1x1_fwd(dy, wt, dx, M, K, N)
+        elif join_stats:
+          G = hip.conv1x1_stats_groups(M, K, N)
+          partial = torch.empty((G, 2, K), dtype=torch.float32, device=x.device)
+          join_entry(dy, wt, dx, res, M, N, K, rgeom=rgeom, bn_x=x, bn_scale_shift=lazy.scale_shift,
+                     bn_mean_invstd=lazy.mean_invstd, bn_act=lazy.act, partial=partial)
+          lazy.bwd_stats = (partial, G, dx.data_ptr())
+        elif rgeom is not None:
+          join_entry(dy, wt, dx, res, M, N, K, rgeom=rgeom)
+        elif fuse_stats:
           G = hip.conv1x1_stats_groups(M, K, N)
           partial = torch.empty((G, 2, K), dtype=torch.float32, device=x.device)
           hip.conv1x1_bwd_data_bnstats(dy, wt, dx, x, lazy.scale_shift, lazy.mean_invstd, lazy.act, partial, M, N, K)
@@ -854,14 +875,17 @@
       if join:
         if not second:
           lazy.pending, dx = dx, None
+          lazy.pending_geom = geom if compact else None
         else:
           if res is None:
             dx = dx + lazy.pending
-          lazy.pending = None
+          lazy.pending = lazy.pending_geom = None
     return dx, dw, (dy if has_res else None), None, None, None, None, None, None
 
 
 JOIN_TWO_CONSUMERS = os.environ.get('PF_JOIN_TWO_CONSUMERS', '1') != '0'
+PROJ_JOIN = os.environ.get('PF_PROJ_JOIN', '1') != '0'
+PROJ_JOIN_STATS = os.environ.get('PF_PROJ_JOIN_STATS', '1') != '0'
 USE_SEG_TRANSPOSE = os.environ.get('PF_SEG_TRANSPOSE', '1') != '0'
 OWN_POOL = os.environ.get('PF_OWN_POOL', '1') != '0'
 OWN_CONV2D_WRW = os.environ.get('PF_OWN_CONV2D_WRW', '1') != '0'
@@ -1281,6 +1305,8 @@
       if torch.is_grad_enabled() and (xin.requires_grad or w.requires_grad):
         if lazy is not None and xin.requires_grad:
           lazy.n_grad_consumers += 1
+          if self.stride == 1:
+            lazy.dense_out = int(w.shape[0])
         return _apply_with_stats(_FusedConv1x1, xin, w, residual, lazy, want_stats, self.stride, self.graph, self.kernel)
       w2d = w.detach().permute(0, 2, 3, 1).reshape(w.shape[0], w.shape[1])
       return _run_conv1x1(xin, w2d, lazy, _nhwc(residual) if residual is not None else None, want_stats,
diff --git a/pocketflow_amd/hip.py b/pocketflow_amd/hip.py
--- a/pocketflow_amd/hip.py
+++ b/pocketflow_amd/hip.py
@@ -44,6 +44,7 @@
     'pf_conv2d_bwd_data_strided_bnstats',
     'pf_cpr_gather', 'pf_cpr_gram_ws', 'pf_cpr_gram', 'pf_cpr_ista', 'pf_cpr_lstsq_splits', 'pf_cpr_lstsq_step', 'pf_cpr_lstsq_resid',
     'pf_conv_gather_fwd',
+    'pf_conv1x1_join_plan', 'pf_conv1x1_bwd_data_join',
 ]
 
 
@@ -451,6 +452,20 @@
                                           c_int(N), c_int(K), _stream()), 'pf_conv1x1_bwd_data_bnstats')
 
 
+def conv1x1_join_plan(M: int, N: int, K: int, with_stats: bool = False) -> int:
+  return int(_lib.pf_conv1x1_join_plan(c_int(M), c_int(N), c_int(K), c_int(1 if with_stats else 0)))
+
+
+def conv1x1_bwd_data_join(dY, Wt, dQ, R, M: int, N: int, K: int, rgeom=None, bn_x=None, bn_scale_shift=None,
+                          bn_mean_invstd=None, bn_act=None, partial=None) -> None:
+  _dev(dY)
+  Ho, Wo, H, Wd, stride = rgeom if rgeom is not None else (0, 0, 0, 0, 1)
+  _check(_lib.pf_conv1x1_bwd_data_join(_ptr(dY), _ptr(Wt), _ptr(dQ), _ptr(R), c_int(Ho), c_int(Wo), c_int(H), c_int(Wd),
+                                       c_int(stride), _ptr(bn_x), _ptr(bn_scale_shift), _ptr(bn_mean_invstd),
+                                       c_int(ACT_CODES[bn_act]), _ptr(partial), c_int(M), c_int(N), c_int(K), _stream()),
+         'pf_conv1x1_bwd_data_join')
+
+
 
 _zero_page = {}
 
```

Result: faster. 11540 (median of 6 runs) (+1.4%).
